# ethz-asl/aerial_mapper

Hardware: AMD Instinct MI355X
Metric: Mcells/s (DSM+ortho) (higher is better)
Workload: dtype f64

## Files before the change

### aerial_mapper_amd/csrc/amhip_api.hip

```cpp
#include <cmath>
#include <cstdio>
#include <cstdlib>
#include <cstring>
#include <limits>
#include <new>

#include "amhip_common.h"

namespace amhip {

static thread_local std::string g_last_error;

void set_last_error(const std::string& msg) { g_last_error = msg; }

int hip_fail(hipError_t e, const char* what, const char* file, int line) {
  char buf[512];
  std::snprintf(buf, sizeof(buf), "HIP error %d (%s) in `%s` at %s:%d", (int)e,
                hipGetErrorString(e), what, file, line);
  set_last_error(buf);
  return e == hipErrorOutOfMemory ? AMHIP_ERR_NOMEM : AMHIP_ERR_HIP;
}

static int arg_fail(const char* msg) {
  set_last_error(msg);
// ... 576 lines not shown
    ay = c.cone_ay;
    if (!tuning_on("no_distorted_prune")) p.r_in = c.cone_rin;
    if (tuning_on("distorted_square_cull")) ax = ay = cone;
  }
  if (have_cone) {
    p.cull = 1;
    double l[3] = {1.0, 0.0, ax}, r[3] = {-1.0, 0.0, ax};
    double t[3] = {0.0, 1.0, ay}, b[3] = {0.0, -1.0, ay};
    normalize3(l);
    normalize3(r);
    normalize3(t);
    normalize3(b);
    for (int k = 0; k < 3; ++k) {
      p.pl[0][k] = l[k];
      p.pl[1][k] = r[k];
      p.pl[2][k] = t[k];
      p.pl[3][k] = b[k];
    }
  } else if (p.cull) {
    const double W = cam.width, H = cam.height;
    double l[3] = {cam.fu, 0.0, cam.cu};
    double r[3] = {-cam.fu, 0.0, W - cam.cu};
    double t[3] = {0.0, cam.fv, cam.cv};
    double b[3] = {0.0, -cam.fv, H - cam.cv};
    normalize3(l);
    normalize3(r);
    normalize3(t);
    normalize3(b);
    for (int k = 0; k < 3; ++k) {
      p.pl[0][k] = l[k];
      p.pl[1][k] = r[k];
      p.pl[2][k] = t[k];
      p.pl[3][k] = b[k];
    }
  }
  *out = p;
}

static float layer_init_value(int layer) {
  switch (layer) {
    case AMHIP_LAYER_ORTHO:
      return 255.0f;
    case AMHIP_LAYER_ELEVATION_ANGLE:
    case AMHIP_LAYER_NUM_OBSERVATIONS:
      return 0.0f;
    default:
      return std::numeric_limits<float>::quiet_NaN();
  }
}

static int use_device(Ctx* c) {
  AMHIP_TRY(hipSetDevice(c->device));
  return AMHIP_OK;
}

static int fetch_status(Ctx* c) {
  AMHIP_TRY(hipMemcpyAsync(c->host_err, c->dev_err, sizeof(unsigned),
                           hipMemcpyDeviceToHost, c->stream));
  AMHIP_TRY(hipMemsetAsync(c->dev_err, 0, sizeof(unsigned), c->stream));
  AMHIP_TRY(hipStreamSynchronize(c->stream));
  const unsigned e = *c->host_err;
  if (e & kDevErrExactHit) {
    set_last_error(
        "a point coincides with a cell centre (reference: dsm.cc:165 "
        "CHECK(distances[i] > 0.0))");
    return AMHIP_ERR_EXACT_HIT;
  }
  if (e & kDevErrAlphaNonPos) {
    set_last_error(
        "observation angle alpha <= 0 (reference: ortho-backward-grid.cc:178 "
        "CHECK(alpha > 0.0))");
    return AMHIP_ERR_ALPHA_NONPOS;
  }
  if (e & kDevErrRectifyZeroW) {
    set_last_error("rectification: w == 0 (reference: rectifier.cpp:93,99 CHECK_NE(xyw(2), 0.0))");
    return AMHIP_ERR_ARG;
  }
  if (e & kDevErrHaloOverflow) {
    set_last_error(
        "tiled DSM: more halo points for a neighbouring window than send rows were reserved "
        "(cap_per_dest): the elevation near that edge is incomplete");
    return AMHIP_ERR_HALO_OVERFLOW;
  }
  return AMHIP_OK;
}

__global__ void k_halo_overflow_check(const unsigned long long* __restrict__ counts, int nd,
                                      unsigned long long cap, unsigned* __restrict__ dev_err) {
  if ((int)threadIdx.x < nd && counts[threadIdx.x] > cap) atomicOr(dev_err, kDevErrHaloOverflow);
}

static bool valid_layer(int l) { return l >= 0 && l < AMHIP_NUM_LAYERS; }

}

using namespace amhip;

extern "C" {

int amhip_abi_version(void) { return AMHIP_ABI_VERSION; }

const char* amhip_last_error(void) { return g_last_error.c_str(); }

void amhip_make_grid(double length_x, double length_y, double resolution,
                     double pos_x, double pos_y, amhip_grid_desc* out) {
  if (!out) return;
  out->rows = static_cast<int>(std::round(length_x / resolution));
  out->cols = static_cast<int>(std::round(length_y / resolution));
  out->resolution = resolution;
  out->length_x = static_cast<double>(out->rows) * resolution;
  out->length_y = static_cast<double>(out->cols) * resolution;
  out->pos_x = pos_x;
  out->pos_y = pos_y;
}

void amhip_cell_position(const amhip_grid_desc* grid, int i, int j, double* x,
                         double* y) {
  double bx, by;
  grid_bases(*grid, &bx, &by);
  if (x) *x = bx + grid->resolution * (-static_cast<double>(i));
  if (y) *y = by + grid->resolution * (-static_cast<double>(j));
}

int amhip_ctx_create(const amhip_grid_desc* grid, int device, amhip_ctx** out) {
  if (!grid) return arg_fail("amhip_ctx_create: null argument");
  return amhip_ctx_create_window(grid, 0, 0, grid->rows, grid->cols, device, out);
}

int amhip_ctx_create_window(const amhip_grid_desc* grid, int i0, int j0, int rows, int cols,
                            int device, amhip_ctx** out) {
  if (!grid || !out) return arg_fail("amhip_ctx_create: null argument");
  if (grid->rows <= 0 || grid->cols <= 0 || !(grid->resolution > 0.0))
    return arg_fail("amhip_ctx_create: empty grid");
  if (i0 < 0 || j0 < 0 || rows <= 0 || cols <= 0 || i0 + rows > grid->rows ||
      j0 + cols > grid->cols)
    return arg_fail("amhip_ctx_create_window: window outside the map");
  *out = nullptr;
  int ndev = 0;
  if (hipGetDeviceCount(&ndev) != hipSuccess || ndev <= 0) {
    (void)hipGetLastError();
    set_last_error("no HIP device visible (libaerial_mapper_hip needs a gfx950 GPU)");
    return AMHIP_ERR_NO_DEVICE;
  }
  if (device < 0 || device >= ndev) return arg_fail("amhip_ctx_create: bad device index");
  amhip_ctx* h = new (std::nothrow) amhip_ctx();
  if (!h) return AMHIP_ERR_NOMEM;
  Ctx* c = &h->impl;
  c->grid = *grid;
  c->device = device;
  c->win_i0 = i0;
  c->win_j0 = j0;
  c->win_rows = rows;
  c->win_cols = cols;
  c->cells = static_cast<size_t>(rows) * static_cast<size_t>(cols);
  {
    c->dsm_exact = amhip_default_dsm_precision() == AMHIP_DSM_EXACT ? 1 : 0;
  }
  int rc = AMHIP_OK;
  do {
    if ((rc = use_device(c))) break;
    if (hipStreamCreateWithFlags(&c->own_stream, hipStreamNonBlocking) != hipSuccess) {
      rc = hip_fail(hipGetLastError(), "hipStreamCreate", __FILE__, __LINE__);
      break;
    }
    c->stream = c->own_stream;
    hipError_t e = hipSuccess;
    for (int l = 0; l < AMHIP_NUM_LAYERS && e == hipSuccess; ++l)
      e = hipMalloc(reinterpret_cast<void**>(&c->layers[l]), c->cells * sizeof(float));
    if (e == hipSuccess) e = hipMalloc(reinterpret_cast<void**>(&c->dev_err), 4 * sizeof(unsigned));
    if (e == hipSuccess)
      e = hipMalloc(reinterpret_cast<void**>(&c->dev_zrange), 4 * sizeof(unsigned long long));
    if (e == hipSuccess)
      e = hipHostMalloc(reinterpret_cast<void**>(&c->host_err), sizeof(unsigned), 0);
    if (e == hipSuccess) {
      e = hipHostMalloc(reinterpret_cast<void**>(&c->host_tile_stats), 8 * sizeof(unsigned), 0);
      if (e == hipSuccess) std::memset(c->host_tile_stats, 0, 8 * sizeof(unsigned));
    }
    if (e == hipSuccess) {
      e = hipHostMalloc(reinterpret_cast<void**>(&c->host_sort_stats), 4 * sizeof(unsigned), 0);
      if (e == hipSuccess) std::memset(c->host_sort_stats, 0xFF, 4 * sizeof(unsigned));
    }
    if (e == hipSuccess) e = hipMalloc(reinterpret_cast<void**>(&c->dev_tickets), 16 * sizeof(unsigned));
    if (e == hipSuccess) e = hipMemsetAsync(c->dev_tickets, 0, 16 * sizeof(unsigned), c->stream);
    if (e == hipSuccess) e = hipMalloc(reinterpret_cast<void**>(&c->dev_bbox), 8 * sizeof(int));
    if (e == hipSuccess) e = hipHostMalloc(reinterpret_cast<void**>(&c->host_bbox), 8 * sizeof(int), 0);
    if (e == hipSuccess) e = hipMemsetAsync(c->dev_err, 0, sizeof(unsigned), c->stream);
    if (e != hipSuccess) {
      rc = hip_fail(e, "context allocation", __FILE__, __LINE__);
      break;
    }
    rc = amhip_layers_reset(h);
  } while (0);
  if (rc != AMHIP_OK) {
    const std::string keep = g_last_error;
    amhip_ctx_destroy(h);
    set_last_error(keep);
    return rc;
  }
  *out = h;
  return AMHIP_OK;
}

void amhip_ctx_destroy(amhip_ctx* h) {
  if (!h) return;
  Ctx* c = &h->impl;
  (void)hipSetDevice(c->device);
  if (c->stream) (void)hipStreamSynchronize(c->stream);
  drain_timers(c);
  for (TimedRegion& r : c->free_regions) {
    (void)hipEventDestroy(r.a);
    (void)hipEventDestroy(r.b);
  }
  for (int l = 0; l < AMHIP_NUM_LAYERS; ++l)
    if (c->layers[l]) (void)hipFree(c->layers[l]);
  void* bufs[] = {c->dev_bbox, c->ortho_list, c->zpart, c->dev_zrange, c->tile_list, c->tile_occ, c->fill_mask, c->stage_values, c->dev_err, c->sorted,       c->rank,        c->bin_start, c->bin_z, c->rec_a, c->rec_b, c->rec16, c->sidx, c->zref, c->zall, c->tmp_points, c->stripe_ws,
                  c->scan_partials, c->stage_points, c->frame_poses, c->stage_frames, c->stereo_ws};
  for (void* b : bufs)
    if (b) (void)hipFree(b);
  jpeg_scratch_free(&c->jpeg);
  if (c->host_err) (void)hipHostFree(c->host_err);
  if (c->host_tile_stats) (void)hipHostFree(c->host_tile_stats);
  if (c->host_sort_stats) (void)hipHostFree(c->host_sort_stats);
  if (c->dev_tickets) (void)hipFree(c->dev_tickets);
  if (c->host_bbox) (void)hipHostFree(c->host_bbox);
  if (c->order_event) (void)hipEventDestroy(c->order_event);
  if (c->own_stream) (void)hipStreamDestroy(c->own_stream);
  delete h;
}

int amhip_ctx_set_dsm_precision(amhip_ctx* h, int mode) {
  if (!h) return arg_fail("null context");
  if (mode != AMHIP_DSM_FAST && mode != AMHIP_DSM_EXACT) return arg_fail("unknown DSM precision mode");
  h->impl.dsm_exact = mode == AMHIP_DSM_EXACT ? 1 : 0;
  return AMHIP_OK;
}

int amhip_ctx_set_dsm_knn(amhip_ctx* h, int k) {
  if (!h) return arg_fail("null context");
  if (k < 0 || k > 8) return arg_fail("amhip_ctx_set_dsm_knn: k must be 0 (off) .. 8");
  h->impl.dsm_knn = k;
  return AMHIP_OK;
}

int amhip_ctx_set_stream(amhip_ctx* h, void* hip_stream) {
  if (!h) return arg_fail("null context");
  Ctx* c = &h->impl;
  int rc = use_device(c);
  if (rc) return rc;
  AMHIP_TRY(hipStreamSynchronize(c->stream));
  c->stream = hip_stream ? static_cast<hipStream_t>(hip_stream) : c->own_stream;
  return AMHIP_OK;
}

int amhip_ctx_synchronize(amhip_ctx* h) {
  if (!h) return arg_fail("null context");
  Ctx* c = &h->impl;
  int rc = use_device(c);
  if (rc) return rc;
  return fetch_status(c);
}

int amhip_layers_reset(amhip_ctx* h) {
  if (!h) return arg_fail("null context");
  Ctx* c = &h->impl;
  int rc = use_device(c);
  if (rc) return rc;
  const bool eager = tuning_on("eager_reset");
  {
    static const unsigned long long empty[2] = {0xFFF0000000000000ull, 0x000FFFFFFFFFFFFFull};
    AMHIP_TRY(hipMemcpyAsync(c->dev_zrange, empty, sizeof(empty), hipMemcpyHostToDevice, c->stream));
    c->zrange_valid = true;
  }
  for (int l = 0; l < AMHIP_NUM_LAYERS; ++l) {
    unsigned char& st = c->layer_state[l];
    if (st == 0 || st == 3) continue;
    if (st == 1 && !eager) {
      st = 3;
      continue;
    }
    if ((rc = launch_fill(c, c->layers[l], c->cells, layer_init_value(l)))) return rc;
    if (st == 1) st = 0;
  }
  return AMHIP_OK;
}

static int materialize(Ctx* c, int layer) {
  if (c->layer_state[layer] != 3) return AMHIP_OK;
  const int rc = launch_fill(c, c->layers[layer], c->cells, layer_init_value(layer));
  if (rc) return rc;
  c->layer_state[layer] = 0;
  return AMHIP_OK;
}

static void dirty_full(Ctx* c) {
  c->dirty_on_device = false;
  c->dirty[0] = c->dirty[1] = 0;
  c->dirty[2] = c->win_rows;
  c->dirty[3] = c->win_cols;
}

static int touch(Ctx* c, int layer) {
  dirty_full(c);
  const int rc = materialize(c, layer);
  if (rc) return rc;
  if (c->layer_state[layer] == 0) c->layer_state[layer] = 1;
  return AMHIP_OK;
// ... 526 lines not shown
                                        observation_index, colored_ortho};
  for (int l = 0; l < AMHIP_NUM_LAYERS; ++l)
    if (ups[l]) {
      overwrite(c, l);
      AMHIP_TRY(hipMemcpyAsync(c->layers[l], ups[l], bytes, hipMemcpyHostToDevice,
                               c->stream));
    }
  const size_t row = (size_t)cam->width * (size_t)channels;
  const size_t frame = row * (size_t)cam->height;
  if ((rc = ensure_capacity(&c->stage_frames, &c->stage_frames_cap, frame * F))) return rc;
  for (size_t f = 0; f < F; ++f) {
    if (!images[f]) return arg_fail("null image");
    if (steps[f] < row) return arg_fail("image step smaller than a row");
    if (steps[f] == row)
      AMHIP_TRY(hipMemcpyAsync(c->stage_frames + f * frame, images[f], frame,
                               hipMemcpyHostToDevice, c->stream));
    else
      AMHIP_TRY(hipMemcpy2DAsync(c->stage_frames + f * frame, row, images[f], steps[f],
                                 row, (size_t)cam->height, hipMemcpyHostToDevice,
                                 c->stream));
  }
  if ((rc = amhip_ortho_backward_process_dev(h, cam, host_T_G_C, F, c->stage_frames,
                                             frame, row, channels, colored)))
    return rc;
  float* downs[AMHIP_NUM_LAYERS] = {ortho,           nullptr,
                                    elevation_angle, num_observations,
                                    observation_index, colored_ortho};
  for (int l = 0; l < AMHIP_NUM_LAYERS; ++l)
    if (downs[l]) {
      if ((rc = materialize(c, l))) return rc;
      AMHIP_TRY(hipMemcpyAsync(downs[l], c->layers[l], bytes, hipMemcpyDeviceToHost,
                               c->stream));
    }
  return fetch_status(c);
}


int amhip_ctx_enable_timing(amhip_ctx* h, int on) {
  if (!h) return arg_fail("null context");
  h->impl.timing = on != 0;
  return AMHIP_OK;
}

int amhip_ctx_timing_reset(amhip_ctx* h) {
  if (!h) return arg_fail("null context");
  Ctx* c = &h->impl;
  int rc = use_device(c);
  if (rc) return rc;
  drain_timers(c);
  for (int k = 0; k < AMHIP_NUM_KERNELS; ++k) {
    c->slot_ms[k] = 0.0;
    c->slot_launches[k] = 0;
  }
  return AMHIP_OK;
}

int amhip_ctx_kernel_time(amhip_ctx* h, int kernel, double* total_ms,
                          int64_t* launches) {
  if (!h || kernel < 0 || kernel >= AMHIP_NUM_KERNELS) return arg_fail("bad kernel slot");
  Ctx* c = &h->impl;
  int rc = use_device(c);
  if (rc) return rc;
  drain_timers(c);
  if (total_ms) *total_ms = c->slot_ms[kernel];
  if (launches) *launches = c->slot_launches[kernel];
  return AMHIP_OK;
}

const char* amhip_kernel_name(int kernel) {
  switch (kernel) {
    case AMHIP_K_DSM_BIN_COUNT:
      return "k_dsm_p3_count";
    case AMHIP_K_DSM_SCATTER:
      return "k_dsm_p3_scatter";
    case AMHIP_K_DSM_SCAN:
      return "k_dsm_p3_place";
    case AMHIP_K_DSM_GATHER:
      return "k_dsm_gather";
    case AMHIP_K_ORTHO:
      return "k_ortho_backward";
    case AMHIP_K_MISC:
      return "memset/fill";
    case AMHIP_K_HALO_SELECT:
      return "k_halo_select";
    case AMHIP_K_STEREO:
      return "k_stereo";
    default:
      return "?";
  }
}

int amhip_set_tuning(const char* key, double value) {
  if (!tuning_set(key, value)) return arg_fail("amhip_set_tuning: unknown key (include/aerial_mapper_hip.h lists them)");
  return AMHIP_OK;
}

double amhip_get_tuning(const char* key, double dflt) { return key ? tuning(key, dflt) : dflt; }

int amhip_default_dsm_precision(void) {
  const char* fast = std::getenv("AMHIP_DSM_FAST");
  return (fast && fast[0] && fast[0] != '0' && !std::getenv("AMHIP_DSM_EXACT")) ? AMHIP_DSM_FAST : AMHIP_DSM_EXACT;
}

int amhip_ctx_order_after(amhip_ctx* h, void* other_stream) {
  if (!h) return arg_fail("null context");
  Ctx* c = &h->impl;
  int rc = use_device(c);
  if (rc) return rc;
  hipStream_t other = static_cast<hipStream_t>(other_stream);
  if (other == c->stream) return AMHIP_OK;
  if (!c->order_event) AMHIP_TRY(hipEventCreateWithFlags(&c->order_event, hipEventDisableTiming));
  AMHIP_TRY(hipEventRecord(c->order_event, c->stream));
  AMHIP_TRY(hipStreamWaitEvent(other, c->order_event, 0));
  return AMHIP_OK;
}

int amhip_ctx_dsm_gather_stats(amhip_ctx* h, int64_t* out8) {
  if (!h || !out8) return arg_fail("amhip_ctx_dsm_gather_stats: null argument");
  Ctx* c = &h->impl;
  int rc = use_device(c);
  if (rc) return rc;
  for (int k = 0; k < 8; ++k) out8[k] = 0;
  if (!c->tile_list || c->last_ntiles == 0) return AMHIP_OK;
  unsigned hdr[8];
  AMHIP_TRY(hipMemcpyAsync(hdr, c->tile_list, sizeof(hdr), hipMemcpyDeviceToHost, c->stream));
  AMHIP_TRY(hipStreamSynchronize(c->stream));
  for (int k = 0; k < 7; ++k) out8[k] = hdr[k];
  out8[4] += hdr[7];
  out8[7] = c->last_ntiles;
  return AMHIP_OK;
}

int amhip_ctx_dsm_stats(amhip_ctx* h, int64_t* points_binned, int64_t* num_bins,
                        int32_t* bin_cells) {
  if (!h) return arg_fail("null context");
  Ctx* c = &h->impl;
  int rc = use_device(c);
  if (rc) return rc;
  if (points_binned) {
    *points_binned = 0;
    if (c->bin_start && c->last_num_bins > 0) {
      uint32_t total = 0;
      AMHIP_TRY(hipMemcpyAsync(&total, c->bin_start + c->last_num_bins,
                               sizeof(uint32_t), hipMemcpyDeviceToHost, c->stream));
      AMHIP_TRY(hipStreamSynchronize(c->stream));
      *points_binned = total;
    }
  }
  if (num_bins) *num_bins = c->last_num_bins;
  if (bin_cells) *bin_cells = c->last_bin_cells;
  return AMHIP_OK;
}

}
```

### aerial_mapper_amd/csrc/amhip_common.h

```cpp
#ifndef AMHIP_COMMON_H_
#define AMHIP_COMMON_H_

#include <hip/hip_runtime.h>

#include <cstddef>
#include <cstdint>
#include <string>
#include <vector>

#include "aerial_mapper_hip.h"
#include "amhip_tuning.h"
#include "amhip_ortho_fold.h"

namespace amhip {

void set_last_error(const std::string& msg);
int hip_fail(hipError_t e, const char* what, const char* file, int line);

#define AMHIP_TRY(expr)                                                  \
  do {                                                                   \
    hipError_t _e = (expr);                                              \
    if (_e != hipSuccess) return ::amhip::hip_fail(_e, #expr, __FILE__, __LINE__); \
  } while (0)

constexpr int kMaxLevels = 24;
constexpr int kMaxW0 = 16;

struct DsmParams {
  double base_x, base_y, res;
  int rows, cols;
  int i_off, j_off;
  double sub_x, sub_y;
  int pcl_mode;
  int only_unfilled;
  double inv_res;
  int B, M, nbx, nby;
  int nlevels;
  double T[kMaxLevels];
  int w[kMaxLevels];
  int lds_ok;
  int p3_r1;
  int p3_c, p3_w;
  int p3_n1, p3_n2;
  int p3_cap;
  unsigned mul_B, mul_r1, mul_w;
  int wr[2 * kMaxW0 + 1];
  int wr2[2 * kMaxW0 + 2];
  int wrp[kMaxW0 + 1];
  int lds_cap;
  int lds_cells;
  int tile_j;
  int tiles_i, tiles_j;
  unsigned lds_bytes;
  int knn_k;
  int fx_ok;
  int fx_S;
  float fx_thi, fx_tlo;
  float fx_denmax;
  float fx_epsw;
  unsigned lds_bytes_f32;
  int canon_all;
  int out_i0, out_j0, out_pitch;
};

struct PtsView {
  const double* sorted;
  const uint4* rec;
  const uint32_t* sidx;
  const double* cloud;
  const double* zref;
  double sub_x, sub_y;
};


struct OrthoParams {
  double base_x, base_y, res;
  int rows, cols;
  int i_off, j_off;
  double fu, fv, cu, cv;
  double dist[4];
  int width, height, distortion;
  int num_frames;
  int channels, colored;
  size_t frame_stride, row_step;
  double pl[4][3];
  int cull;
  int virt_out, virt_nobs;
  int coarse;
  int fast;
  FoldCam fold;
  int prune;
  double radius_scale;
  double r_in;
};

enum : unsigned { kDevErrExactHit = 1u, kDevErrAlphaNonPos = 2u, kDevErrHaloOverflow = 4u,
                  kDevErrRectifyZeroW = 8u };

constexpr int kMaxHaloDests = 8;
struct HaloParams {
  double base_x, base_y, inv_res, sub_x, sub_y;
  int nd;
  double lo_i[kMaxHaloDests], hi_i[kMaxHaloDests], lo_j[kMaxHaloDests], hi_j[kMaxHaloDests];
  unsigned long long cap;
  unsigned long long off[kMaxHaloDests], cap_d[kMaxHaloDests];
  double in_lo_i, in_hi_i, in_lo_j, in_hi_j;
};
struct SortSplit {
  int phase;
  size_t n_prefix;
  HaloParams hp;
  double* halo_out;
  unsigned long long* halo_counts;
};

struct JpegScratch {
  uint8_t* dev = nullptr;
  size_t cap = 0;
  uint8_t* pinned = nullptr;
  uint8_t* image = nullptr;
  size_t image_cap = 0;
  uint8_t* out = nullptr;
  size_t out_cap = 0;
};
enum { kJpegGray8 = 0, kJpegBgr8 = 1, kJpegBgr16s = 2 };
struct JpegSource {
  const void* dev;
  size_t step;
  int width, height;
  int mode;
};
void jpeg_scratch_free(JpegScratch* ws);
int jpeg_scratch_image(JpegScratch* ws, size_t bytes, uint8_t** out);
int jpeg_encode_run(hipStream_t stream, JpegScratch* ws, const JpegSource& src, int quality,
                    uint8_t* dev_out, size_t cap, size_t* bytes);
int jpeg_write_run(const char* what, hipStream_t stream, JpegScratch* ws, const JpegSource& src,
                   int quality, const char* filename);

struct TimedRegion {
  hipEvent_t a, b;
  int slot;
};

struct Ctx {
  amhip_grid_desc grid;
  int win_i0 = 0, win_j0 = 0;
  int win_rows = 0, win_cols = 0;
  int device = 0;
  hipStream_t own_stream = nullptr;
  hipStream_t stream = nullptr;
  hipEvent_t order_event = nullptr;
  size_t cells = 0;
  int dsm_exact = 0;
  int dsm_exact_now = 0;
  int rough_hold = 0;
  bool last_call_f32 = false;
  int dsm_knn = 0;

  float* layers[AMHIP_NUM_LAYERS] = {nullptr, nullptr, nullptr,
                                     nullptr, nullptr, nullptr};
  unsigned char layer_state[AMHIP_NUM_LAYERS] = {1, 1, 1, 1, 1, 1};
  unsigned long long* dev_zrange = nullptr;
  bool zrange_valid = false;
  double* zpart = nullptr;
  size_t zpart_cap = 0;
  unsigned* dev_err = nullptr;
  unsigned* host_err = nullptr;

  PtsView pts = {};
  double* sorted = nullptr;
  size_t sorted_cap = 0;
  uint32_t* rank = nullptr;
  size_t rank_cap = 0;
  uint32_t* bin_start = nullptr;
  size_t bin_cap = 0;
  uint32_t* rec_a = nullptr;
  size_t rec_a_cap = 0;
  uint32_t* rec_b = nullptr;
  size_t rec_b_cap = 0;
  uint32_t* rec16 = nullptr;
  size_t rec16_cap = 0;
  uint32_t* sidx = nullptr;
  size_t sidx_cap = 0;
  double* zref = nullptr;
  size_t zref_cap = 0;
  double* zall = nullptr;
  size_t zall_cap = 0;
  uint32_t* bin_z = nullptr;
  size_t bin_z_cap = 0;
  bool bin_z_valid = false;
  uint32_t* scan_partials = nullptr;
  size_t partial_cap = 0;
  double* tmp_points = nullptr;
  size_t tmp_points_cap = 0;
  uint32_t* stripe_ws = nullptr;
  size_t stripe_ws_cap = 0;
  uint8_t* tile_occ = nullptr;
  size_t tile_occ_cap = 0;
  int* tile_list = nullptr;
  size_t tile_list_cap = 0;
  unsigned char* fill_mask = nullptr;
  size_t fill_mask_cap = 0;
  int32_t* stage_values = nullptr;
  size_t stage_values_cap = 0;
  double* stage_points = nullptr;
  size_t stage_points_cap = 0;

  amhip_camera cone_cam = {};
  double cone = 0.0;
  int cone_state = 0;
  int cone_state_rect = 0;
  double cone_rect_cone = 0.0, cone_ax = 0.0, cone_ay = 0.0, cone_rin = 0.0;
  FramePose* frame_poses = nullptr;
  size_t frame_pose_cap = 0;
  uint8_t* stage_frames = nullptr;
  size_t stage_frames_cap = 0;
  int dirty[4] = {0, 0, 0, 0};
  bool dirty_on_device = false;
  int* dev_bbox = nullptr;
  int* host_bbox = nullptr;
  int* ortho_list = nullptr;
  size_t ortho_list_cap = 0;

  bool tiled_pending = false;
  const double* tiled_xyz = nullptr;
  size_t tiled_n = 0;
  int tiled_radius_sq = 0;
  double tiled_ce = 0.0, tiled_cn = 0.0;
  SortSplit tiled_split = {};
  DsmParams tiled_params = {};

  int64_t last_points_binned = 0;
  int64_t last_num_bins = 0;
  int32_t last_bin_cells = 0;
  int64_t last_ntiles = 0;
  uint32_t* aux_zero_words = nullptr;
  int aux_nzero = 0;
  bool aux_done = false;
  size_t range_parts = 0;
  unsigned long long* range_running = nullptr;
  unsigned* dev_tickets = nullptr;
  unsigned* host_sort_stats = nullptr;
  unsigned long long sort_stats_sig = 0, tile_stats_sig = 0;
  unsigned* host_tile_stats = nullptr;

  uint8_t* stereo_ws = nullptr;
  size_t stereo_ws_cap = 0;
  JpegScratch jpeg;

  bool timing = false;
  std::vector<TimedRegion> regions;
  std::vector<TimedRegion> free_regions;
  double slot_ms[AMHIP_NUM_KERNELS] = {};
  int64_t slot_launches[AMHIP_NUM_KERNELS] = {};
};

struct ScopedTimer {
  Ctx* c;
  TimedRegion r;
  bool on;
  ScopedTimer(Ctx* ctx, int slot);
  ~ScopedTimer();
};

template <typename T>
int ensure_capacity(T** ptr, size_t* cap, size_t need);

int ensure_bytes(void** ptr, size_t* cap_bytes, size_t need_bytes);

int launch_fill(Ctx* c, float* dst, size_t n, float value);

struct DensifyParams {
  int width, height;
  size_t disp_step, img_step;
  double Q03, Q11, Q13, Q23, Q32;
  double R[9], t[3];
};
inline DensifyParams densify_params(const double* K, double baseline, const double* R_G_C,
                                    const double* t_G_C1, int width, int height, size_t disp_step,
                                    size_t img_step) {
  DensifyParams p = {};
  p.width = width;
  p.height = height;
  p.disp_step = disp_step;
  p.img_step = img_step;
  const double fx = K[0], fy = K[4], cx = K[2], cy = K[5];
  p.Q03 = -cx;
  p.Q11 = fx / fy;
  p.Q13 = -cy * (fx / fy);
  p.Q23 = fx;
  p.Q32 = 1.0 / baseline;
  for (int k = 0; k < 9; ++k) p.R[k] = R_G_C[k];
  for (int k = 0; k < 3; ++k) p.t[k] = t_G_C1[k];
  return p;
}
int densify_run(Ctx* c, const DensifyParams& p, const float* dev_disparity,
                const uint8_t* dev_image_left, double* dev_xyz_out, int32_t* dev_intensity_out,
                size_t capacity, long long* dev_count);

struct SeqState {
  unsigned long long running, base;
  unsigned pairs, skip;
};
int densify_append_run(Ctx* c, const DensifyParams& p, const float* dev_disparity,
                       const uint8_t* dev_image_left, double* dev_xyz, int32_t* dev_intensities,
                       size_t capacity, SeqState* dev_state, void* dev_pc2, bool replace,
                       const unsigned* dev_err_word = nullptr);
struct BatchStrides {
  size_t left, right, mask, disp, raw;
};
struct StereoImages {
  const uint8_t* left;
  size_t left_step;
  const uint8_t* right;
  size_t right_step;
  const uint8_t* mask;
  size_t mask_step;
  float* disp;
  size_t disp_step;
  int16_t* raw;
  size_t raw_step;
  int batch;
  BatchStrides bs;
};
int stereo_params_check(const amhip_stereo_settings& s, int width, int height);
int stereo_scratch_reserve(Ctx* c, const amhip_stereo_settings& s, int width, int height, int batch);
int stereo_match(Ctx* c, const amhip_stereo_settings& s, int width, int height, const StereoImages& im);
int undistort_frames_run(hipStream_t stream, const amhip_camera& cam, const uint8_t* dev_frames,
                         size_t frame_stride, size_t row_step, int channels, int G, uint8_t* dev_out);

int halo_select_run(Ctx* c, const double* dev_xyz, size_t n, const HaloParams& hp,
                    double* dev_out, unsigned long long* dev_counts);
constexpr int kBboxBias = 1 << 30;
int dsm_bbox_run(Ctx* c, const double* dev_xyz, size_t n, const DsmParams& p, int* dev_bbox5);
int make_halo_params(const Ctx& c, double center_easting, double center_northing,
                     const int32_t* dest_windows, int nd, double margin_m, size_t cap_per_dest,
                     HaloParams* out);
bool no_launch_skips();
int dsm_sort(Ctx* c, const double* dev_xyz, const int32_t* dev_values, size_t n,
             const DsmParams& p, unsigned long long* zrange, const SortSplit* split = nullptr);
int dsm_run(Ctx* c, const double* dev_xyz, const int32_t* dev_values, size_t n,
            const DsmParams& p, float* out, unsigned char* mask, unsigned* unfilled,
            bool fill_untouched = false, float init_value = 0.0f,
            unsigned long long* zrange = nullptr, const SortSplit* split = nullptr);
int ortho_run(Ctx* c, const OrthoParams& p, const FramePose* dev_poses, const FrameFast* dev_fast,
              const uint8_t* dev_frames);

int ctx_last_dirty(Ctx* c, int rect[4]);
int ctx_use_device(Ctx* c);
int ctx_materialize(Ctx* c, int layer);
void ctx_overwrite(Ctx* c, int layer);
int ctx_layer_set_initial(Ctx* c, int layer);
int ctx_fetch_status(Ctx* c);
float ctx_layer_init_value(int layer);
bool ctx_layer_is_initial(const Ctx* c, int layer);
int arg_failure(const char* msg);

struct HPose {
  double qw, qx, qy, qz, tx, ty, tz;
};
HPose hpose_from7(const double* p);
HPose hpose_inverse(const HPose& T);
HPose hpose_compose(const HPose& A, const HPose& B);

}

struct amhip_ctx {
  amhip::Ctx impl;
};

#endif
```

### aerial_mapper_amd/csrc/amhip_sort.hip

```cpp
#include <algorithm>
#include <cstdlib>

#include "amhip_common.h"
#include "amhip_device.h"

namespace amhip {

constexpr uint32_t kNoRank = 0xFFFFFFFFu;

__device__ __forceinline__ int div_by(int n, int d, unsigned m) {
  if (m == 0u) return n;
  if (m == 0xFFFFFFFFu) return n / d;
  return (int)__umulhi((unsigned)n, m);
}

__device__ __forceinline__ bool point_bin(const DsmParams& p, double px,
                                          double py, uint32_t* bin) {
  const double cx = (p.base_x - px) * p.inv_res - (double)p.i_off;
  const double cy = (p.base_y - py) * p.inv_res - (double)p.j_off;
  const double lo = -(double)p.M - 0.5;
  const double hx = (double)(p.rows + p.M) - 0.5;
  const double hy = (double)(p.cols + p.M) - 0.5;
  if (!(cx >= lo && cx < hx && cy >= lo && cy < hy)) return false;
  int ix = (int)floor(cx + 0.5) + p.M;
// ... 236 lines not shown
          if (zall) {
            zlo = fmin(zlo, z[u]);
            zhi = fmax(zhi, z[u]);
          }
        }
        if (kHalo && halo_candidate(hp, x[u], y[u])) look |= 1u << u;
      }
    }
    if (kHalo) {
#pragma nounroll
      while (look) {
        const int u = __builtin_ctz(look);
        look &= look - 1;
        halo_emit(stage, hp, xyz, base + (size_t)u * stride, halo_out, halo_counts);
      }
    }
  }
  if (kHalo) halo_flush(stage, hp, xyz, halo_out, halo_counts);
  if (zall)
    range_commit_wave(zlo, zhi, zall, (size_t)blockIdx.x * (kP3CountThreads / 64) + (threadIdx.x >> 6));
  __syncthreads();
  uint32_t* row = hist_rows + (size_t)blockIdx.x * nk;
  for (int k = threadIdx.x; k < nk; k += kP3CountThreads) row[k] = s_hist[k];
}

struct SortAux {
  unsigned long long* call_range;
  uint32_t* zero_words;
  int nzero;
};
__device__ __forceinline__ void aux_reset(const SortAux& a) {
  if (threadIdx.x == 0 && a.call_range) {
    a.call_range[0] = kOrderedPlusInf;
    a.call_range[1] = kOrderedMinusInf;
  }
  if (a.zero_words && (int)threadIdx.x < a.nzero) a.zero_words[threadIdx.x] = 0u;
}

__device__ __forceinline__ void
p3_scan_body(const uint32_t* __restrict__ cnt, int n1, int n2,
              uint32_t* __restrict__ start2, uint32_t* __restrict__ cursor2,
              uint32_t* __restrict__ start1, uint32_t* __restrict__ cursor1,
              uint32_t* __restrict__ blk2, unsigned cap_small, unsigned cap_big,
              uint32_t* __restrict__ big_list, unsigned chunk,
              unsigned* __restrict__ host_big ) {
  __shared__ unsigned lds[1024 / 64 + 1];
  __shared__ unsigned s_start1[kP3MaxKeys + 1];
  const int nk = n1 * n2;
  unsigned carry = 0;
  if (threadIdx.x == 0) big_list[0] = 0;
  __syncthreads();
  constexpr int kMaxIt = 32;
  {
    const int lane = threadIdx.x & 63, wid = threadIdx.x >> 6;
    const int seg = ((nk + 16 * 64 - 1) / (16 * 64)) * 64;
    const int iters = seg / 64;
    const int w0 = wid * seg;
    unsigned v[kMaxIt];
#pragma unroll
    for (int q = 0; q < kMaxIt; ++q) {
      const int i = w0 + q * 64 + lane;
      v[q] = (q < iters && i < nk) ? cnt[i] : 0u;
    }
    unsigned run = 0;
#pragma unroll
    for (int q = 0; q < kMaxIt; ++q) {
      if (q < iters) {
        if (v[q] > cap_small)
          big_list[1 + atomicAdd(&big_list[0], 1u)] = (uint32_t)(w0 + q * 64 + lane);
        const unsigned incl = wave_incl_scan(v[q], lane);
        v[q] = run + incl - v[q];
        run += __shfl(incl, 63, 64);
      }
    }
    if (lane == 0) lds[wid] = run;
    __syncthreads();
    unsigned base = 0, total = 0;
#pragma unroll
    for (int w = 0; w < 16; ++w) {
      const unsigned t = lds[w];
      if (w < wid) base += t;
      total += t;
    }
#pragma unroll
    for (int q = 0; q < kMaxIt; ++q) {
      const int i = w0 + q * 64 + lane;
      if (q < iters && i < nk) {
        const unsigned st = base + v[q];
        start2[i] = st;
        cursor2[i] = st;
        if (i % n2 == 0) s_start1[i / n2] = st;
      }
    }
    carry = total;
  }
  __syncthreads();
  if (threadIdx.x == 0) {
    start2[nk] = carry;
    s_start1[n1] = carry;
  }
  __syncthreads();
  const int k = threadIdx.x;
  unsigned nblk = 0;
  if (k < n1) {
    start1[k] = s_start1[k];
    cursor1[k] = s_start1[k];
    nblk = (s_start1[k + 1] - s_start1[k] + chunk - 1) / chunk;
  }
  if (k == 0) start1[n1] = carry;
  unsigned total;
  const unsigned ex = block_excl_scan<1024>(nblk, &total, lds);
  if (k < n1) blk2[k] = ex;
  if (k == 0) blk2[n1] = total;
  if (k == 0 && host_big) host_big[0] = big_list[0];
}

__global__ void __launch_bounds__(1024)
k_dsm_p3_reduce_scan(const uint32_t* __restrict__ hist_rows, int nrows, uint32_t* __restrict__ cnt, int n1, int n2,
                     uint32_t* __restrict__ start2, uint32_t* __restrict__ cursor2,
                     uint32_t* __restrict__ start1, uint32_t* __restrict__ cursor1,
                     uint32_t* __restrict__ blk2, unsigned cap_small, unsigned cap_big,
                     uint32_t* __restrict__ big_list, unsigned chunk,
                     SortAux aux, unsigned* __restrict__ host_big, unsigned* __restrict__ ticket) {
  __shared__ uint32_t s_part[16][64];
  __shared__ unsigned s_last;
  const int nk = n1 * n2;
  const int lane = threadIdx.x & 63, wid = threadIdx.x >> 6;
  const int k = blockIdx.x * 64 + lane;
  uint32_t sum = 0;
  if (k < nk)
    for (int r = wid; r < nrows; r += 16) sum += hist_rows[(size_t)r * nk + k];
  s_part[wid][lane] = sum;
  __syncthreads();
  if (wid == 0 && k < nk) {
    uint32_t t = 0;
#pragma unroll
    for (int w = 0; w < 16; ++w) t += s_part[w][lane];
    cnt[k] = t;
  }
  __syncthreads();
  if (threadIdx.x == 0) {
    __threadfence();
    s_last = atomicAdd(ticket, 1u) == gridDim.x - 1u ? 1u : 0u;
  }
  __syncthreads();
  if (!s_last) return;
  __threadfence();
  if (threadIdx.x == 0) *ticket = 0u;
  aux_reset(aux);
  p3_scan_body(cnt, n1, n2, start2, cursor2, start1, cursor1, blk2, cap_small, cap_big, big_list, chunk, host_big);
}


template <bool kFirst>
__device__ __forceinline__ void p3_scatter_body(const unsigned vb, const double* __restrict__ src,
                                                const int32_t* __restrict__ values, size_t n,
                                                const DsmParams& p, const uint32_t* __restrict__ start1,
                                                const uint32_t* __restrict__ blk2,
                                                uint32_t* __restrict__ cursor, double* __restrict__ dst,
                                                double* __restrict__ zpart) {
  extern __shared__ double s_pts[];
  uint32_t* s_dest = reinterpret_cast<uint32_t*>(s_pts + 3 * kP3Chunk);
  uint32_t* s_cnt = s_dest + kP3Chunk;
  uint32_t* s_off = s_cnt + kP3MaxKeys;
  uint32_t* s_base = s_off + kP3MaxKeys;
  uint32_t* s_scan = s_base + kP3MaxKeys;
  const int tid = threadIdx.x;
  int nkeys;
  size_t c0, c1;
  if (kFirst) {
    c0 = (size_t)vb * kP3Chunk;
    c1 = min(c0 + (size_t)kP3Chunk, n);
    nkeys = p.p3_n1;
  } else {
    const int n1 = p.p3_n1;
    const uint32_t b = vb;
    if (b >= blk2[n1]) return;
    int lo = 0, hi = n1;
    while (hi - lo > 1) {
      const int mid = (lo + hi) >> 1;
      if (blk2[mid] <= b) lo = mid; else hi = mid;
    }
    c0 = (size_t)start1[lo] + (size_t)(b - blk2[lo]) * kP3Chunk;
    c1 = min(c0 + (size_t)kP3Chunk, (size_t)start1[lo + 1]);
    nkeys = p.p3_n2;
    cursor += (size_t)lo * p.p3_n2;
  }
  if (tid < kP3MaxKeys) s_cnt[tid] = 0;
  __syncthreads();
  double px[kP3PerThread], py[kP3PerThread], pz[kP3PerThread];
  double zlo = __builtin_huge_val(), zhi = -__builtin_huge_val();
  uint32_t slot[kP3PerThread];
  if (c1 <= c0) return;
#pragma unroll
  for (int k = 0; k < kP3PerThread; ++k) {
    const size_t ld = min(c0 + tid + (size_t)k * kP3Threads, c1 - 1);
    px[k] = src[3 * ld + 0];
    py[k] = src[3 * ld + 1];
    pz[k] = src[3 * ld + 2];
  }
  if (kFirst && values) {
#pragma unroll
    for (int k = 0; k < kP3PerThread; ++k)
      pz[k] = (double)values[min(c0 + tid + (size_t)k * kP3Threads, c1 - 1)];
  }
#pragma unroll
  for (int k = 0; k < kP3PerThread; ++k) {
    const size_t idx = c0 + tid + (size_t)k * kP3Threads;
    slot[k] = 0xFFFFFFFFu;
    if (idx < c1) {
      double x = px[k], y = py[k];
      const double z = pz[k];
      if (kFirst) {
        x -= p.sub_x;
        y -= p.sub_y;
      }
      px[k] = x;
      py[k] = y;
      int k1, k2;
      if (p3_keys(p, x, y, &k1, &k2)) {
        const int key = kFirst ? k1 : k2;
        slot[k] = ((uint32_t)key << 13) | atomicAdd(&s_cnt[key], 1u);
        if (kFirst) {
          zlo = fmin(zlo, z);
          zhi = fmax(zhi, z);
        }
      }
    }
  }
  if (kFirst && zpart)
    range_commit_wave(zlo, zhi, zpart, (size_t)vb * (kP3Threads / 64) + (tid >> 6));
  __syncthreads();
  unsigned my_base = 0;
  {
    const unsigned c = (tid < nkeys) ? s_cnt[tid] : 0u;
    unsigned total;
    const unsigned ex = block_excl_scan<kP3Threads>(c, &total, s_scan);
    if (tid < nkeys) {
      s_off[tid] = ex;
      if (c) my_base = atomicAdd(&cursor[tid], c);
    }
    if (tid == 0) s_scan[23] = total;
  }
  __syncthreads();
#pragma unroll
  for (int k = 0; k < kP3PerThread; ++k) {
    if (slot[k] != 0xFFFFFFFFu) {
      const uint32_t key = slot[k] >> 13, rank = slot[k] & 0x1FFFu;
      const uint32_t q = s_off[key] + rank;
      s_pts[3 * q + 0] = px[k];
      s_pts[3 * q + 1] = py[k];
      s_pts[3 * q + 2] = pz[k];
      s_dest[q] = slot[k];
    }
  }
  if (tid < nkeys) s_base[tid] = my_base;
  __syncthreads();
  const uint32_t ne = 3u * s_scan[23];
  for (uint32_t e = tid; e < ne; e += kP3Threads) {
    const uint32_t q = e / 3u;
    const uint32_t d = s_dest[q];
    const uint32_t b = s_base[d >> 13];
    dst[3 * (size_t)(b + (d & 0x1FFFu)) + (e - 3u * q)] = s_pts[e];
  }
}

template <bool kFirst>
__global__ void __launch_bounds__(kP3Threads)
k_dsm_p3_scatter(const double* __restrict__ src, const int32_t* __restrict__ values, size_t n,
                 DsmParams p, const uint32_t* __restrict__ start1,
                 const uint32_t* __restrict__ blk2, uint32_t* __restrict__ cursor,
                 double* __restrict__ dst, double* __restrict__ zpart) {
  p3_scatter_body<kFirst>(blockIdx.x, src, values, n, p, start1, blk2, cursor, dst, zpart);
}

__device__ __forceinline__ uint32_t place_zkey(double z) {
  const uint32_t b = __float_as_uint((float)z);
  return (b >> 31) ? ~b : (b | 0x80000000u);
}
template <int THREADS, int PER>
__device__ __forceinline__ void place_subpartition(const double* __restrict__ src, const DsmParams& p,
                                                   int cap, const uint32_t* __restrict__ start2,
                                                   uint32_t* __restrict__ bin_start,
                                                   double* __restrict__ sorted, int sp,
                                                   unsigned skip_lo, unsigned skip_hi,
                                                   uint2* __restrict__ bin_z) {
  extern __shared__ double s_pts[];
  uint32_t* s_bins = reinterpret_cast<uint32_t*>(s_pts + 3 * cap);
  uint32_t* s_scan = s_bins + p.p3_w;
  uint32_t* s_zlo = s_scan + 24;
  uint32_t* s_zhi = s_zlo + p.p3_w;
  const int tid = threadIdx.x;
  const int k1 = sp / p.p3_n2, k2 = sp - k1 * p.p3_n2;
  const int rr = k2 / p.p3_c;
  const int row = k1 * p.p3_r1 + rr;
  const int bx0 = (k2 - rr * p.p3_c) * p.p3_w;
  const int nbw = min(p.p3_w, p.nbx - bx0);
  if (sp == 0 && tid == 0)
    bin_start[(size_t)p.nbx * p.nby] = start2[p.p3_n1 * p.p3_n2];
  if (row >= p.nby || nbw <= 0) return;
  const uint32_t g0 = start2[sp], g1 = start2[sp + 1];
  for (int k = tid; k < nbw; k += THREADS) {
    s_bins[k] = 0;
    if (bin_z) {
      s_zlo[k] = 0xFFFFFFFFu;
      s_zhi[k] = 0u;
    }
  }
  __syncthreads();
  if ((g1 - g0) > skip_lo && (g1 - g0) <= skip_hi) return;
  const bool in_lds = (int)(g1 - g0) <= cap && cap <= THREADS * PER;
  double px[PER], py[PER], pz[PER];
  int pb[PER];
  if (in_lds) {
    if (g1 > g0) {
#pragma unroll
      for (int k = 0; k < PER; ++k) {
        const size_t ld = min(g0 + tid + (uint32_t)k * THREADS, g1 - 1);
        px[k] = src[3 * ld + 0];
        py[k] = src[3 * ld + 1];
        pz[k] = src[3 * ld + 2];
      }
    }
#pragma unroll
    for (int k = 0; k < PER; ++k) {
      const uint32_t idx = g0 + tid + (uint32_t)k * THREADS;
      pb[k] = -1;
      if (idx < g1) {
        int bx, by;
        point_bin_xy(p, px[k], py[k], &bx, &by);
        pb[k] = bx - bx0;
        atomicAdd(&s_bins[pb[k]], 1u);
        if (bin_z) {
          const uint32_t zk = place_zkey(pz[k]);
          atomicMin(&s_zlo[pb[k]], zk);
          atomicMax(&s_zhi[pb[k]], zk);
        }
      }
    }
  } else {
    for (uint32_t idx = g0 + tid; idx < g1; idx += THREADS) {
      int bx, by;
      point_bin_xy(p, src[3 * (size_t)idx + 0], src[3 * (size_t)idx + 1], &bx, &by);
      atomicAdd(&s_bins[bx - bx0], 1u);
    }
  }
  __syncthreads();
  {
    const int per = (nbw + THREADS - 1) / THREADS;
    const int lo = tid * per;
    const int hi = min(lo + per, nbw);
    unsigned sum = 0;
    for (int k = lo; k < hi; ++k) sum += s_bins[k];
    unsigned total;
    unsigned run = block_excl_scan<THREADS>(sum, &total, s_scan);
    for (int k = lo; k < hi; ++k) {
      const unsigned t = s_bins[k];
      s_bins[k] = run;
      run += t;
    }
  }
  __syncthreads();
  uint32_t* out_start = bin_start + (size_t)row * p.nbx + bx0;
  for (int k = tid; k < nbw; k += THREADS) out_start[k] = g0 + s_bins[k];
  if (bin_z && in_lds) {
    uint2* zrow = bin_z + (size_t)row * p.nbx + bx0;
    for (int k = tid; k < nbw; k += THREADS) zrow[k] = make_uint2(s_zlo[k], s_zhi[k]);
  }
  __syncthreads();
  if (!in_lds) {
    for (uint32_t idx = g0 + tid; idx < g1; idx += THREADS) {
      const double x = src[3 * (size_t)idx + 0];
      const double y = src[3 * (size_t)idx + 1];
      const double z = src[3 * (size_t)idx + 2];
      int bx, by;
      point_bin_xy(p, x, y, &bx, &by);
      const size_t o = (size_t)g0 + atomicAdd(&s_bins[bx - bx0], 1u);
      sorted[3 * o + 0] = x;
      sorted[3 * o + 1] = y;
      sorted[3 * o + 2] = z;
      if (bin_z) {
        const uint32_t zk = place_zkey(z);
        atomicMin(&s_zlo[bx - bx0], zk);
        atomicMax(&s_zhi[bx - bx0], zk);
      }
    }
    if (bin_z) {
      __syncthreads();
      uint2* zrow = bin_z + (size_t)row * p.nbx + bx0;
      for (int k = tid; k < nbw; k += THREADS) zrow[k] = make_uint2(s_zlo[k], s_zhi[k]);
    }
    return;
  }
#pragma unroll
  for (int k = 0; k < PER; ++k) {
    if (pb[k] >= 0) {
      const uint32_t q = atomicAdd(&s_bins[pb[k]], 1u);
      s_pts[3 * q + 0] = px[k];
      s_pts[3 * q + 1] = py[k];
      s_pts[3 * q + 2] = pz[k];
    }
  }
  __syncthreads();
  const uint32_t ne = 3u * (g1 - g0);
  double* out = sorted + 3 * (size_t)g0;
  for (uint32_t e = tid; e < ne; e += THREADS) out[e] = s_pts[e];
}


template <int THREADS, bool kRec, int PER>
__device__ __forceinline__ void place_rounds(const void* __restrict__ src_v, const DsmParams& p, int cap,
                                             const uint32_t* __restrict__ start2,
                                             uint32_t* __restrict__ bin_start, double* __restrict__ sorted,
                                             uint4* __restrict__ rec16, uint32_t* __restrict__ sidx,
                                             uint2* __restrict__ bin_z, int sp) {
  extern __shared__ double s_pts_raw[];
  constexpr int kWordsPer = kRec ? 5 : 6;
  constexpr int kRegs = PER > 0 ? PER : 1;
  uint32_t* s_words = reinterpret_cast<uint32_t*>(s_pts_raw);
  uint32_t* s_bins = s_words + (size_t)kWordsPer * cap;
  uint32_t* s_cur = s_bins + p.p3_w + 1;
  uint32_t* s_scan = s_cur + p.p3_w;
  uint32_t* s_zlo = s_scan + 24;
  uint32_t* s_zhi = s_zlo + p.p3_w;
  const double* srcd = reinterpret_cast<const double*>(src_v);
  const uint32_t* srcw = reinterpret_cast<const uint32_t*>(src_v);
  const int tid = threadIdx.x;
  const int k1 = sp / p.p3_n2, k2 = sp - k1 * p.p3_n2;
  const int rr = k2 / p.p3_c;
  const int row = k1 * p.p3_r1 + rr;
  const int bx0 = (k2 - rr * p.p3_c) * p.p3_w;
  const int nbw = min(p.p3_w, p.nbx - bx0);
  if (row >= p.nby || nbw <= 0) return;
  const uint32_t g0 = start2[sp], g1 = start2[sp + 1];
  auto zkey = [](uint32_t fbits) { return (fbits >> 31) ? ~fbits : (fbits | 0x80000000u); };
  for (int k = tid; k <= nbw; k += THREADS) s_bins[k] = 0;
  if (bin_z)
    for (int k = tid; k < nbw; k += THREADS) {
      s_zlo[k] = 0xFFFFFFFFu;
      s_zhi[k] = 0u;
    }
  __syncthreads();
  auto bin_of = [&](uint32_t idx) -> int {
    if (kRec) return div_by((int)(srcw[(size_t)kRecWords * idx] & 0xFFFFu), p.B, p.mul_B) - bx0;
    int bx, by;
    point_bin_xy(p, srcd[3 * (size_t)idx + 0], srcd[3 * (size_t)idx + 1], &bx, &by);
    return bx - bx0;
  };
  double rx[kRegs], ry[kRegs], rz[kRegs];
  uint32_t rw[kRegs][kRecWords];
  int rb[kRegs];
  if (PER > 0) {
    if (g1 > g0) {
#pragma unroll
      for (int k = 0; k < kRegs; ++k) {
        const size_t ld = min(g0 + tid + (uint32_t)k * THREADS, g1 - 1);
        if (kRec) {
#pragma unroll
          for (int t = 0; t < kRecWords; ++t) rw[k][t] = srcw[(size_t)kRecWords * ld + t];
        } else {
          rx[k] = srcd[3 * ld + 0];
          ry[k] = srcd[3 * ld + 1];
          rz[k] = srcd[3 * ld + 2];
        }
      }
    }
#pragma unroll
    for (int k = 0; k < kRegs; ++k) {
      const uint32_t idx = g0 + tid + (uint32_t)k * THREADS;
      rb[k] = -1;
      if (idx < g1) {
        if (kRec) {
          rb[k] = div_by((int)(rw[k][0] & 0xFFFFu), p.B, p.mul_B) - bx0;
        } else {
          int bx, by;
          point_bin_xy(p, rx[k], ry[k], &bx, &by);
          rb[k] = bx - bx0;
        }
        atomicAdd(&s_bins[rb[k]], 1u);
        if (bin_z) {
          const uint32_t zk = kRec ? zkey(rw[k][3]) : place_zkey(rz[k]);
          atomicMin(&s_zlo[rb[k]], zk);
          atomicMax(&s_zhi[rb[k]], zk);
        }
      }
    }
  } else {
    for (uint32_t idx = g0 + tid; idx < g1; idx += THREADS) {
      const int b = bin_of(idx);
      atomicAdd(&s_bins[b], 1u);
      if (bin_z) {
        const uint32_t zk = kRec ? zkey(srcw[(size_t)kRecWords * idx + 3]) : place_zkey(srcd[3 * (size_t)idx + 2]);
        atomicMin(&s_zlo[b], zk);
        atomicMax(&s_zhi[b], zk);
      }
    }
  }
  __syncthreads();
  {
    const int per = (nbw + THREADS - 1) / THREADS;
    const int lo = tid * per;
    const int hi = min(lo + per, nbw);
    unsigned sum = 0;
    for (int k = lo; k < hi; ++k) sum += s_bins[k];
    unsigned total;
    unsigned run = block_excl_scan<THREADS>(sum, &total, s_scan);
    for (int k = lo; k < hi; ++k) {
      const unsigned t = s_bins[k];
      s_bins[k] = run;
      run += t;
    }
    if (tid == 0) s_bins[nbw] = total;
  }
  __syncthreads();
  {
    uint32_t* out_start = bin_start + (size_t)row * p.nbx + bx0;
    for (int k = tid; k < nbw; k += THREADS) out_start[k] = g0 + s_bins[k];
    if (bin_z) {
      uint2* zrow = bin_z + (size_t)row * p.nbx + bx0;
      for (int k = tid; k < nbw; k += THREADS) zrow[k] = make_uint2(s_zlo[k], s_zhi[k]);
    }
  }
  auto put = [&](bool direct, uint32_t q, uint32_t base, const uint32_t* v, double x, double y, double z) {
    if (kRec) {
      if (direct) {
        rec16[(size_t)g0 + q] = make_uint4(v[0], v[1], v[2], v[3]);
        sidx[(size_t)g0 + q] = v[4];
      } else {
#pragma unroll
        for (int t = 0; t < kRecWords; ++t) s_words[(size_t)kRecWords * (q - base) + t] = v[t];
      }
    } else {
      double* o = direct ? sorted + 3 * ((size_t)g0 + q) : s_pts_raw + 3 * (size_t)(q - base);
      o[0] = x;
      o[1] = y;
      o[2] = z;
    }
  };
  int lo_bin = 0;
  while (lo_bin < nbw) {
    const uint32_t base = s_bins[lo_bin];
    int a = lo_bin, b = nbw;
    while (b - a > 0) {
      const int mid = (a + b + 1) >> 1;
      if (s_bins[mid] - base <= (uint32_t)cap) a = mid; else b = mid - 1;
    }
    const bool direct = a == lo_bin;
    const int hi_bin = direct ? lo_bin + 1 : a;
    const uint32_t cnt = s_bins[hi_bin] - base;
    for (int k = lo_bin + tid; k < hi_bin; k += THREADS) s_cur[k] = s_bins[k];
    __syncthreads();
    if (PER > 0) {
#pragma unroll
      for (int k = 0; k < kRegs; ++k) {
        if (rb[k] >= lo_bin && rb[k] < hi_bin) {
          const uint32_t q = atomicAdd(&s_cur[rb[k]], 1u);
          put(direct, q, base, rw[k], rx[k], ry[k], rz[k]);
        }
      }
    } else {
      for (uint32_t idx = g0 + tid; idx < g1; idx += THREADS) {
        const int bb = bin_of(idx);
        if (bb < lo_bin || bb >= hi_bin) continue;
        const uint32_t q = atomicAdd(&s_cur[bb], 1u);
        uint32_t v[kRecWords] = {0u, 0u, 0u, 0u, 0u};
        double x = 0.0, y = 0.0, z = 0.0;
        if (kRec) {
#pragma unroll
          for (int t = 0; t < kRecWords; ++t) v[t] = srcw[(size_t)kRecWords * idx + t];
        } else {
          x = srcd[3 * (size_t)idx + 0];
          y = srcd[3 * (size_t)idx + 1];
          z = srcd[3 * (size_t)idx + 2];
        }
        put(direct, q, base, v, x, y, z);
      }
    }
    __syncthreads();
    if (!direct) {
      if (kRec) {
        for (uint32_t q = tid; q < cnt; q += THREADS) {
          const uint32_t* r = s_words + (size_t)kRecWords * q;
          rec16[(size_t)g0 + base + q] = make_uint4(r[0], r[1], r[2], r[3]);
          sidx[(size_t)g0 + base + q] = r[4];
        }
      } else {
        double* out = sorted + 3 * ((size_t)g0 + base);
        for (uint32_t e = tid; e < 3u * cnt; e += THREADS) out[e] = s_pts_raw[e];
      }
    }
    __syncthreads();
    lo_bin = hi_bin;
  }
}

__global__ void __launch_bounds__(kP3PlaceThreads)
k_dsm_p3_place(const double* __restrict__ src, DsmParams p, int cap,
               const uint32_t* __restrict__ start2, uint32_t* __restrict__ bin_start,
               double* __restrict__ sorted, unsigned skip_lo, unsigned skip_hi,
               uint2* __restrict__ bin_z,
               const uint32_t* __restrict__ big_list, unsigned* __restrict__ host_big) {
  if (host_big && blockIdx.x == 0 && threadIdx.x == 0) host_big[0] = big_list[0];
  place_subpartition<kP3PlaceThreads, kP3PlacePer>(src, p, cap, start2, bin_start, sorted,
                                                   (int)blockIdx.x, skip_lo, skip_hi, bin_z);
}

__global__ void __launch_bounds__(kP3BigThreads)
k_dsm_p3_place_big(const double* __restrict__ src, DsmParams p,
                   const uint32_t* __restrict__ start2, uint32_t* __restrict__ bin_start,
                   double* __restrict__ sorted, const uint32_t* __restrict__ big_list,
                   uint2* __restrict__ bin_z, int cap_rounds, unsigned rounds_above, unsigned reg_max) {
  const unsigned count = big_list[0];
  for (unsigned k = blockIdx.x; k < count; k += gridDim.x) {
    const int sp = (int)big_list[1 + k];
    const uint32_t cnt = start2[sp + 1] - start2[sp];
    if (cnt > rounds_above && cnt <= min(reg_max, (unsigned)(kP3BigThreads * kP3RoundsPer)))
      place_rounds<kP3BigThreads, false, kP3RoundsPer>(src, p, cap_rounds, start2, bin_start, sorted, nullptr,
                                                       nullptr, bin_z, sp);
    else if (cnt > rounds_above)
      place_rounds<kP3BigThreads, false, 0>(src, p, cap_rounds, start2, bin_start, sorted, nullptr, nullptr,
                                            bin_z, sp);
    else
      place_subpartition<kP3BigThreads, kP3BigPer>(src, p, kP3BigCap, start2, bin_start, sorted, sp, 0u,
                                                   0u, bin_z);
    __syncthreads();
  }
}

constexpr int kRecPerThread = 6;
constexpr int kRecChunk = kP3Threads * kRecPerThread;

__global__ void __launch_bounds__(1024)
k_dsm_zref(const double* __restrict__ part, size_t nparts, double* __restrict__ zref) {
  __shared__ double s_pair[2 * 16];
  double lo = __builtin_huge_val(), hi = -__builtin_huge_val();
  for (size_t k = threadIdx.x; k < nparts; k += 1024) {
    lo = fmin(lo, part[2 * k]);
    hi = fmax(hi, part[2 * k + 1]);
  }
#pragma unroll
  for (int d = 32; d > 0; d >>= 1) {
    lo = fmin(lo, __shfl_xor(lo, d, 64));
    hi = fmax(hi, __shfl_xor(hi, d, 64));
  }
  if ((threadIdx.x & 63) == 0) {
    s_pair[2 * (threadIdx.x >> 6)] = lo;
    s_pair[2 * (threadIdx.x >> 6) + 1] = hi;
  }
  __syncthreads();
  if (threadIdx.x == 0) {
    for (int w = 1; w < 16; ++w) {
      lo = fmin(lo, s_pair[2 * w]);
      hi = fmax(hi, s_pair[2 * w + 1]);
    }
    const bool ok = lo <= hi && lo > -1.0e300 && hi < 1.0e300;
    zref[0] = ok ? 0.5 * lo + 0.5 * hi : 0.0;
    zref[1] = lo;
    zref[2] = hi;
  }
}

__device__ __forceinline__ bool make_record(const DsmParams& p, double px, double py, double z,
                                            double zref, uint32_t row, uint32_t* w) {
  const double cx = (p.base_x - px) * p.inv_res - (double)p.i_off;
  const double cy = (p.base_y - py) * p.inv_res - (double)p.j_off;
  const double lo = -(double)p.M - 0.5;
  const double hx = (double)(p.rows + p.M) - 0.5;
  const double hy = (double)(p.cols + p.M) - 0.5;
  if (!(cx >= lo && cx < hx && cy >= lo && cy < hy)) return false;
  int ix = (int)floor(cx + 0.5) + p.M;
  int iy = (int)floor(cy + 0.5) + p.M;
  ix = min(max(ix, 0), p.rows + 2 * p.M - 1);
  iy = min(max(iy, 0), p.cols + 2 * p.M - 1);
  const double scale = (double)(1u << p.fx_S);
  const double fx = (cx + (double)p.M) - (double)ix;
  const double fy = (cy + (double)p.M) - (double)iy;
  w[0] = (uint32_t)ix | ((uint32_t)iy << 16);
  w[1] = (uint32_t)(int)rint(fx * scale);
  w[2] = (uint32_t)(int)rint(fy * scale);
  w[3] = __float_as_uint((float)(z - zref));
  w[4] = row;
  return true;
}

__device__ __forceinline__ void record_keys(const DsmParams& p, uint32_t w0, int* k1, int* k2,
                                            int* bx_out) {
  const int bx = div_by((int)(w0 & 0xFFFFu), p.B, p.mul_B);
  const int by = div_by((int)(w0 >> 16), p.B, p.mul_B);
  const int a = div_by(by, p.p3_r1, p.mul_r1);
  *k1 = a;
  *k2 = (by - a * p.p3_r1) * p.p3_c + div_by(bx, p.p3_w, p.mul_w);
  *bx_out = bx;
}

template <bool kFirst>
__global__ void __launch_bounds__(kP3Threads)
k_dsm_p3_scatter_rec(const double* __restrict__ cloud, const uint32_t* __restrict__ src, size_t n,
                     DsmParams p, const double* __restrict__ zref,
                     const uint32_t* __restrict__ start1, const uint32_t* __restrict__ blk2,
                     uint32_t* __restrict__ cursor, uint32_t* __restrict__ dst,
                     double* __restrict__ zpart) {
  extern __shared__ uint32_t s_words[];
  uint32_t* s_dest = s_words + kRecWords * kRecChunk;
  uint32_t* s_cnt = s_dest + kRecChunk;
  uint32_t* s_off = s_cnt + kP3MaxKeys;
  uint32_t* s_base = s_off + kP3MaxKeys;
  uint32_t* s_scan = s_base + kP3MaxKeys;
  const int tid = threadIdx.x;
  int nkeys;
  size_t c0, c1;
  if (kFirst) {
    c0 = (size_t)blockIdx.x * kRecChunk;
    c1 = min(c0 + (size_t)kRecChunk, n);
    nkeys = p.p3_n1;
  } else {
    const int n1 = p.p3_n1;
    const uint32_t b = blockIdx.x;
    if (b >= blk2[n1]) return;
    int lo = 0, hi = n1;
    while (hi - lo > 1) {
      const int mid = (lo + hi) >> 1;
      if (blk2[mid] <= b) lo = mid; else hi = mid;
    }
    c0 = (size_t)start1[lo] + (size_t)(b - blk2[lo]) * kRecChunk;
    c1 = min(c0 + (size_t)kRecChunk, (size_t)start1[lo + 1]);
    nkeys = p.p3_n2;
    cursor += (size_t)lo * p.p3_n2;
  }
  if (tid < kP3MaxKeys) s_cnt[tid] = 0;
  __syncthreads();
  const double zr = kFirst ? zref[0] : 0.0;
  uint32_t w[kRecPerThread][kRecWords];
  double zlo = __builtin_huge_val(), zhi = -__builtin_huge_val();
  uint32_t slot[kRecPerThread];
  if (c1 <= c0) return;
  double cx[kFirst ? kRecPerThread : 1], cy[kFirst ? kRecPerThread : 1], cz[kFirst ? kRecPerThread : 1];
#pragma unroll
  for (int k = 0; k < kRecPerThread; ++k) {
    const size_t ld = min(c0 + tid + (size_t)k * kP3Threads, c1 - 1);
    if (kFirst) {
      cx[k] = cloud[3 * ld + 0];
      cy[k] = cloud[3 * ld + 1];
      cz[k] = cloud[3 * ld + 2];
    } else {
#pragma unroll
      for (int q = 0; q < kRecWords; ++q) w[k][q] = src[kRecWords * ld + q];
    }
  }
#pragma unroll
  for (int k = 0; k < kRecPerThread; ++k) {
    const size_t idx = c0 + tid + (size_t)k * kP3Threads;
    slot[k] = 0xFFFFFFFFu;
    if (idx < c1) {
      bool in;
      if (kFirst) {
        const double x = cx[k] - p.sub_x;
        const double y = cy[k] - p.sub_y;
        const double z = cz[k];
        in = make_record(p, x, y, z, zr, (uint32_t)idx, w[k]);
        if (in) {
          zlo = fmin(zlo, z);
          zhi = fmax(zhi, z);
        }
      } else {
        in = true;
      }
      if (in) {
        int k1, k2, bx;
        record_keys(p, w[k][0], &k1, &k2, &bx);
        const int key = kFirst ? k1 : k2;
        slot[k] = ((uint32_t)key << 13) | atomicAdd(&s_cnt[key], 1u);
      }
    }
  }
  if (kFirst && zpart)
    range_commit_wave(zlo, zhi, zpart, (size_t)blockIdx.x * (kP3Threads / 64) + (tid >> 6));
  __syncthreads();
// ... 254 lines not shown
    w[2] = lo_j;
    w[3] = hi_j;
    w[4] = (int)cnt;
  }
  __syncthreads();
  if (threadIdx.x == 0) {
    unsigned total = 0;
    for (int k = 0; k < 4; ++k) {
      lo_i = min(lo_i, s_box[k][0]);
      hi_i = max(hi_i, s_box[k][1]);
      lo_j = min(lo_j, s_box[k][2]);
      hi_j = max(hi_j, s_box[k][3]);
      total += (unsigned)s_box[k][4];
    }
    if (total) {
      atomicMax(&out5[0], kBboxBias - lo_i);
      atomicMax(&out5[1], hi_i + kBboxBias);
      atomicMax(&out5[2], kBboxBias - lo_j);
      atomicMax(&out5[3], hi_j + kBboxBias);
      atomicAdd(reinterpret_cast<unsigned*>(&out5[4]), total);
    }
  }
}

int dsm_bbox_run(Ctx* c, const double* dev_xyz, size_t n, const DsmParams& p, int* dev_bbox5) {
  ScopedTimer t(c, AMHIP_K_DSM_BIN_COUNT);
  AMHIP_TRY(hipMemsetAsync(dev_bbox5, 0, 5 * sizeof(int), c->stream));
  size_t grid = std::min<size_t>((n + 2047) / 2048, 128);
  hipLaunchKernelGGL(k_dsm_bbox, dim3((unsigned)grid), dim3(256), 0, c->stream, dev_xyz, n, p, dev_bbox5);
  AMHIP_TRY(hipGetLastError());
  return AMHIP_OK;
}

constexpr int kScanT = 256;
constexpr int kScanI = 16;
constexpr int kScanE = kScanT * kScanI;

__global__ void __launch_bounds__(kScanT)
k_scan_partials(const uint32_t* __restrict__ in, size_t n,
                uint32_t* __restrict__ partials) {
  __shared__ unsigned lds[kScanT / 64 + 1];
  const size_t base = (size_t)blockIdx.x * kScanE + (size_t)threadIdx.x * kScanI;
  unsigned s = 0;
  if (base + kScanI <= n) {
    const uint4* v = reinterpret_cast<const uint4*>(in + base);
#pragma unroll
    for (int k = 0; k < kScanI / 4; ++k) {
      const uint4 q = v[k];
      s += q.x + q.y + q.z + q.w;
    }
  } else {
    for (int k = 0; k < kScanI; ++k)
      if (base + k < n) s += in[base + k];
  }
  unsigned total;
  (void)block_excl_scan<kScanT>(s, &total, lds);
  if (threadIdx.x == 0) partials[blockIdx.x] = total;
}

__global__ void __launch_bounds__(1024)
k_scan_top(uint32_t* __restrict__ partials, size_t nb,
           uint32_t* __restrict__ total_out, SortAux aux) {
  __shared__ unsigned lds[1024 / 64 + 1];
  aux_reset(aux);
  unsigned carry = 0;
  for (size_t base = 0; base < nb; base += 1024) {
    const size_t i = base + threadIdx.x;
    const unsigned v = (i < nb) ? partials[i] : 0u;
    unsigned total;
    const unsigned ex = block_excl_scan<1024>(v, &total, lds);
    if (i < nb) partials[i] = carry + ex;
    carry += total;
  }
  if (threadIdx.x == 0) *total_out = carry;
}

__global__ void __launch_bounds__(kScanT)
k_scan_final(uint32_t* __restrict__ data, size_t n,
             const uint32_t* __restrict__ partials) {
  __shared__ unsigned lds[kScanT / 64 + 1];
  const size_t base = (size_t)blockIdx.x * kScanE + (size_t)threadIdx.x * kScanI;
  unsigned v[kScanI];
  const bool full = base + kScanI <= n;
  if (full) {
    const uint4* src = reinterpret_cast<const uint4*>(data + base);
#pragma unroll
    for (int k = 0; k < kScanI / 4; ++k) {
      const uint4 q = src[k];
      v[4 * k + 0] = q.x;
      v[4 * k + 1] = q.y;
      v[4 * k + 2] = q.z;
      v[4 * k + 3] = q.w;
    }
  } else {
#pragma unroll
    for (int k = 0; k < kScanI; ++k) v[k] = (base + k < n) ? data[base + k] : 0u;
  }
  unsigned s = 0;
#pragma unroll
  for (int k = 0; k < kScanI; ++k) s += v[k];
  unsigned total;
  unsigned run = block_excl_scan<kScanT>(s, &total, lds) + partials[blockIdx.x];
#pragma unroll
  for (int k = 0; k < kScanI; ++k) {
    const unsigned t = v[k];
    v[k] = run;
    run += t;
  }
  if (full) {
    uint4* dst = reinterpret_cast<uint4*>(data + base);
#pragma unroll
    for (int k = 0; k < kScanI / 4; ++k)
      dst[k] = make_uint4(v[4 * k], v[4 * k + 1], v[4 * k + 2], v[4 * k + 3]);
  } else {
#pragma unroll
    for (int k = 0; k < kScanI; ++k)
      if (base + k < n) data[base + k] = v[k];
  }
}


static void p3_rounds_knob(int* cap_rounds, unsigned* rounds_above, unsigned* reg_max) {
  const int knob = (int)tuning("p3_rounds_cap", 0.0);
  const bool reread = tuning_on("p3_rounds_reread");
  if (knob >= 16 && knob < *cap_rounds) {
    *cap_rounds = knob;
    *rounds_above = (unsigned)knob;
  }
  if (reread) *reg_max = 0u;
}

bool no_launch_skips() {
  return tuning_on("no_launch_skips");
}

static unsigned long long sort_geometry_signature(const DsmParams& p) {
  unsigned long long h = 1469598103934665603ull;
  auto mix = [&](const void* v, size_t bytes) {
    const unsigned char* b = static_cast<const unsigned char*>(v);
    for (size_t k = 0; k < bytes; ++k) h = (h ^ b[k]) * 1099511628211ull;
  };
  const int ints[] = {p.rows, p.cols, p.M, p.B, p.nbx, p.nby, p.i_off, p.j_off, p.p3_r1, p.p3_c,
                      p.p3_w, p.p3_n1, p.p3_n2, p.p3_cap};
  const double dbls[] = {p.base_x, p.base_y, p.res, p.inv_res, p.sub_x, p.sub_y};
  mix(ints, sizeof(ints));
  mix(dbls, sizeof(dbls));
  return h ? h : 1ull;
}


static int dsm_sort_impl(Ctx* c, const double* dev_xyz, const int32_t* dev_values, size_t n,
                         const DsmParams& p, unsigned long long* zrange, const SortSplit* split);

int dsm_sort(Ctx* c, const double* dev_xyz, const int32_t* dev_values, size_t n,
             const DsmParams& p, unsigned long long* zrange, const SortSplit* split) {
  const int rc = dsm_sort_impl(c, dev_xyz, dev_values, n, p, zrange, split);
  if (rc) return rc;
  if (!c->aux_done && !(split && split->phase == 1)) return arg_failure("dsm_sort: the call's range was not reset");
  return AMHIP_OK;
}

static int dsm_sort_impl(Ctx* c, const double* dev_xyz, const int32_t* dev_values, size_t n,
                         const DsmParams& p, unsigned long long* zrange, const SortSplit* split) {
  double* zpart = nullptr;
  {
    const size_t max_waves = 8 * std::max<size_t>((n + 2047) / 2048 + 1, 256 * 16);
    const int rc = ensure_capacity(&c->zpart, &c->zpart_cap, 2 * max_waves + 16);
    if (rc) return rc;
    zpart = c->zpart;
  }
  const SortAux aux = {c->dev_zrange + 2, c->aux_zero_words, c->aux_zero_words ? c->aux_nzero : 0};
  c->aux_done = false;
  c->range_parts = 0;
  c->range_running = zrange;
  const size_t nbins = (size_t)p.nbx * (size_t)p.nby;
  const size_t nblocks_scan = (nbins + kScanE - 1) / kScanE;
  const bool force_one_level_ = tuning_on("sort_one_level");
  const unsigned long long geo_sig = sort_geometry_signature(p);
  {
    int rc;
    if ((rc = ensure_capacity(&c->sorted, &c->sorted_cap, 3 * n))) return rc;
    if ((rc = ensure_capacity(&c->bin_start, &c->bin_cap, nbins + 4))) return rc;
  }
  c->last_num_bins = (int64_t)nbins;
  c->last_bin_cells = p.B;
  c->bin_z_valid = false;
  c->pts = PtsView{c->sorted, nullptr, nullptr, dev_xyz, nullptr, p.sub_x, p.sub_y};
  const bool rec = p.fx_ok && !p.pcl_mode && !dev_values;
  if (rec) {
    int rc;
    if ((rc = ensure_capacity(&c->rec16, &c->rec16_cap, 4 * n + 16))) return rc;
    if ((rc = ensure_capacity(&c->sidx, &c->sidx_cap, n + 16))) return rc;
    if ((rc = ensure_capacity(&c->zref, &c->zref_cap, (size_t)8))) return rc;
  }

  const bool force_one_level = force_one_level_;
  const bool three_pass = p.p3_n1 > 0 && !force_one_level;
  if (split && split->phase == 1 && !three_pass)
    return halo_select_run(c, dev_xyz, split->n_prefix, split->hp, split->halo_out,
                           split->halo_counts);
  if (split && !three_pass) split = nullptr;
  if (three_pass) {
    const int n1 = p.p3_n1, n2 = p.p3_n2, nk = n1 * n2;
    auto count_grid = [](size_t len) {
      return std::min<size_t>(std::max<size_t>((len + 8191) / 8192, 1), 256);
    };
    const size_t n_a = split ? split->n_prefix : n;
    const size_t g_a = count_grid(n_a), g_b = n > n_a ? count_grid(n - n_a) : 0;
    const size_t gcount = g_a + g_b;
    int rc;
    if (rec) {
      if ((rc = ensure_capacity(&c->rec_a, &c->rec_a_cap, (size_t)kRecWords * n + 16))) return rc;
      if ((rc = ensure_capacity(&c->rec_b, &c->rec_b_cap, (size_t)kRecWords * n + 16))) return rc;
      if ((rc = ensure_capacity(&c->zall, &c->zall_cap, 2 * gcount * (kP3CountThreads / 64) + 16))) return rc;
    } else if ((rc = ensure_capacity(&c->tmp_points, &c->tmp_points_cap, 3 * n))) {
      return rc;
    }
    double* const zall = rec ? c->zall : nullptr;
    const size_t ws_words = gcount * (size_t)nk + 4 * (size_t)nk + 4 * (size_t)n1 + 64;
    if ((rc = ensure_capacity(&c->stripe_ws, &c->stripe_ws_cap, ws_words))) return rc;
    uint32_t* hist_rows = c->stripe_ws;
    uint32_t* cnt = hist_rows + gcount * (size_t)nk;
    uint32_t* start2 = cnt + nk;
    uint32_t* cursor2 = start2 + nk + 1;
    uint32_t* start1 = cursor2 + nk;
    uint32_t* cursor1 = start1 + n1 + 1;
    uint32_t* blk2 = cursor1 + n1;
    uint32_t* big_list = blk2 + n1 + 1;
    {
      ScopedTimer t(c, AMHIP_K_DSM_BIN_COUNT);
      const size_t lds = (size_t)nk * sizeof(uint32_t);
      const size_t lds_halo = (size_t)((nk + 1) & ~1) * sizeof(uint32_t) + sizeof(HaloStage);
      AMHIP_TRY(hipFuncSetAttribute(reinterpret_cast<const void*>(k_dsm_p3_count<false>),
                                    hipFuncAttributeMaxDynamicSharedMemorySize, (int)lds));
      AMHIP_TRY(hipFuncSetAttribute(reinterpret_cast<const void*>(k_dsm_p3_count<true>),
                                    hipFuncAttributeMaxDynamicSharedMemorySize, (int)lds_halo));
      const HaloParams no_halo = {};
      if (split && split->phase == 1) {
        AMHIP_TRY(hipMemsetAsync(split->halo_counts, 0,
                                 sizeof(unsigned long long) * split->hp.nd, c->stream));
        hipLaunchKernelGGL(k_dsm_p3_count<true>, dim3((unsigned)g_a), dim3(kP3CountThreads),
                           lds_halo, c->stream, dev_xyz, n_a, p, hist_rows, split->hp, split->halo_out,
                           split->halo_counts, zall);
        AMHIP_TRY(hipGetLastError());
        return AMHIP_OK;
      }
      if (!split)
        hipLaunchKernelGGL(k_dsm_p3_count<false>, dim3((unsigned)g_a), dim3(kP3CountThreads), lds,
                           c->stream, dev_xyz, n_a, p, hist_rows, no_halo, (double*)nullptr,
                           (unsigned long long*)nullptr, zall);
      else if (g_b)
        hipLaunchKernelGGL(k_dsm_p3_count<false>, dim3((unsigned)g_b), dim3(kP3CountThreads), lds,
                           c->stream, dev_xyz + 3 * n_a, n - n_a, p, hist_rows + g_a * (size_t)nk,
                           no_halo, (double*)nullptr, (unsigned long long*)nullptr,
                           zall ? zall + 2 * g_a * (kP3CountThreads / 64) : nullptr);
      if (rec)
        hipLaunchKernelGGL(k_dsm_zref, dim3(1), dim3(1024), 0, c->stream, zall,
                           (split && !g_b ? g_a : gcount) * (size_t)(kP3CountThreads / 64), c->zref);
      hipLaunchKernelGGL(k_dsm_p3_reduce_scan, dim3((unsigned)((nk + 63) / 64)), dim3(1024), 0, c->stream,
                         hist_rows, (int)gcount, cnt, n1, n2, start2, cursor2, start1, cursor1, blk2,
                         (unsigned)p.p3_cap, (unsigned)kP3BigCap, big_list, (unsigned)(rec ? kRecChunk : kP3Chunk),
                         aux, (unsigned*)nullptr, c->dev_tickets);
      c->aux_done = true;
      AMHIP_TRY(hipGetLastError());
    }
    if (rec) {
      {
        ScopedTimer t(c, AMHIP_K_DSM_SCATTER);
        const size_t lds = (size_t)kRecChunk * (kRecWords + 1) * 4 + (3 * kP3MaxKeys + 32) * sizeof(uint32_t);
        AMHIP_TRY(hipFuncSetAttribute(reinterpret_cast<const void*>(k_dsm_p3_scatter_rec<true>),
                                      hipFuncAttributeMaxDynamicSharedMemorySize, (int)lds));
        AMHIP_TRY(hipFuncSetAttribute(reinterpret_cast<const void*>(k_dsm_p3_scatter_rec<false>),
                                      hipFuncAttributeMaxDynamicSharedMemorySize, (int)lds));
        const size_t g1 = (n + kRecChunk - 1) / kRecChunk;
        hipLaunchKernelGGL(k_dsm_p3_scatter_rec<true>, dim3((unsigned)g1), dim3(kP3Threads), lds,
                           c->stream, dev_xyz, (const uint32_t*)nullptr, n, p, c->zref, start1, blk2,
                           cursor1, c->rec_a, zpart);
        c->range_parts = (size_t)g1 * (kP3Threads / 64);
        hipLaunchKernelGGL(k_dsm_p3_scatter_rec<false>, dim3((unsigned)(g1 + n1)), dim3(kP3Threads),
                           lds, c->stream, (const double*)nullptr, c->rec_a, n, p, c->zref, start1, blk2,
                           cursor2, c->rec_b, (double*)nullptr);
        AMHIP_TRY(hipGetLastError());
      }
      {
        ScopedTimer t(c, AMHIP_K_DSM_SCAN);
        if ((rc = ensure_capacity(&c->bin_z, &c->bin_z_cap, 2 * (nbins + 4)))) return rc;
        uint2* bin_z = reinterpret_cast<uint2*>(c->bin_z);
        uint4* rec16 = reinterpret_cast<uint4*>(c->rec16);
        const size_t lds = (size_t)p.p3_cap * kRecWords * 4 + (3 * (size_t)p.p3_w + 32) * sizeof(uint32_t);
        AMHIP_TRY(hipFuncSetAttribute(reinterpret_cast<const void*>(k_dsm_p3_place_rec),
                                      hipFuncAttributeMaxDynamicSharedMemorySize, (int)lds));
        hipLaunchKernelGGL(k_dsm_p3_place_rec, dim3((unsigned)nk), dim3(kP3PlaceThreads), lds,
                           c->stream, c->rec_b, p, p.p3_cap, start2, c->bin_start, rec16, c->sidx, bin_z,
                           (unsigned)p.p3_cap, 0xFFFFFFFFu);
        const size_t tables = (4 * (size_t)p.p3_w + 64) * sizeof(uint32_t);
        int cap_rounds = (int)std::min<size_t>(kP3BigCap, (kLdsMaxBytes - tables) / (kRecWords * 4));
        unsigned rounds_above = kP3BigCap, reg_max = 0xFFFFFFFFu;
        p3_rounds_knob(&cap_rounds, &rounds_above, &reg_max);
        const size_t lds_big = std::max((size_t)kP3BigCap * kRecWords * 4 + (3 * (size_t)p.p3_w + 32) * sizeof(uint32_t),
                                        (size_t)cap_rounds * kRecWords * 4 + tables);
        AMHIP_TRY(hipFuncSetAttribute(reinterpret_cast<const void*>(k_dsm_p3_place_rec_big),
                                      hipFuncAttributeMaxDynamicSharedMemorySize, (int)lds_big));
        hipLaunchKernelGGL(k_dsm_p3_place_rec_big, dim3(256), dim3(kP3BigThreads), lds_big, c->stream,
                           c->rec_b, p, start2, c->bin_start, rec16, c->sidx, bin_z, big_list, cap_rounds, rounds_above, reg_max);
        AMHIP_TRY(hipGetLastError());
        c->bin_z_valid = true;
        c->pts = PtsView{nullptr, rec16, c->sidx, dev_xyz, c->zref, p.sub_x, p.sub_y};
      }
      return AMHIP_OK;
    }
    {
      ScopedTimer t(c, AMHIP_K_DSM_SCATTER);
      const size_t lds = (size_t)kP3Chunk * 28 + (3 * kP3MaxKeys + 32) * sizeof(uint32_t);
      AMHIP_TRY(hipFuncSetAttribute(reinterpret_cast<const void*>(k_dsm_p3_scatter<true>),
                                    hipFuncAttributeMaxDynamicSharedMemorySize, (int)lds));
      AMHIP_TRY(hipFuncSetAttribute(reinterpret_cast<const void*>(k_dsm_p3_scatter<false>),
                                    hipFuncAttributeMaxDynamicSharedMemorySize, (int)lds));
      const size_t g1 = (n + kP3Chunk - 1) / kP3Chunk;
      hipLaunchKernelGGL(k_dsm_p3_scatter<true>, dim3((unsigned)g1), dim3(kP3Threads), lds,
                         c->stream, dev_xyz, dev_values, n, p, start1, blk2, cursor1, c->sorted,
                         zpart);
      c->range_parts = (size_t)g1 * (kP3Threads / 64);
      hipLaunchKernelGGL(k_dsm_p3_scatter<false>, dim3((unsigned)(g1 + n1)), dim3(kP3Threads),
                         lds, c->stream, c->sorted, (const int32_t*)nullptr, n, p, start1, blk2,
                         cursor2, c->tmp_points, (double*)nullptr);
      AMHIP_TRY(hipGetLastError());
    }
    {
      ScopedTimer t(c, AMHIP_K_DSM_SCAN);
      uint2* bin_z = nullptr;
      const size_t zlds = bin_z ? 2 * (size_t)p.p3_w * sizeof(uint32_t) : 0;
      const size_t lds = (size_t)p.p3_cap * 24 + ((size_t)p.p3_w + 32) * sizeof(uint32_t) + zlds;
      AMHIP_TRY(hipFuncSetAttribute(reinterpret_cast<const void*>(k_dsm_p3_place),
                                    hipFuncAttributeMaxDynamicSharedMemorySize, (int)lds));
      const bool want_big = !(c->sort_stats_sig == geo_sig && c->host_sort_stats && c->host_sort_stats[0] == 0u) ||
                            no_launch_skips();
      c->sort_stats_sig = geo_sig;
      hipLaunchKernelGGL(k_dsm_p3_place, dim3((unsigned)nk), dim3(kP3PlaceThreads), lds,
                         c->stream, c->tmp_points, p, p.p3_cap, start2, c->bin_start, c->sorted,
                         want_big ? (unsigned)p.p3_cap : 0xFFFFFFFFu, 0xFFFFFFFFu, bin_z,
                         (const uint32_t*)big_list, c->host_sort_stats);
      const size_t tables = (4 * (size_t)p.p3_w + 64) * sizeof(uint32_t);
      int cap_rounds = (int)std::min<size_t>(kP3BigCap, (kLdsMaxBytes - tables) / 24);
      unsigned rounds_above = kP3BigCap, reg_max = 0xFFFFFFFFu;
      p3_rounds_knob(&cap_rounds, &rounds_above, &reg_max);
      const size_t lds_big = std::max((size_t)kP3BigCap * 24 + ((size_t)p.p3_w + 32) * sizeof(uint32_t) + zlds,
                                      (size_t)cap_rounds * 24 + tables);
      AMHIP_TRY(hipFuncSetAttribute(reinterpret_cast<const void*>(k_dsm_p3_place_big),
                                    hipFuncAttributeMaxDynamicSharedMemorySize, (int)lds_big));
      if (want_big)
        hipLaunchKernelGGL(k_dsm_p3_place_big, dim3(256), dim3(kP3BigThreads), lds_big, c->stream,
                           c->tmp_points, p, start2, c->bin_start, c->sorted, big_list, bin_z, cap_rounds, rounds_above, reg_max);
      c->bin_z_valid = bin_z != nullptr;
      AMHIP_TRY(hipGetLastError());
    }
  } else {
    {
      int rc;
      if ((rc = ensure_capacity(&c->rank, &c->rank_cap, n))) return rc;
      if ((rc = ensure_capacity(&c->scan_partials, &c->partial_cap, nblocks_scan + 4))) return rc;
    }
    {
      ScopedTimer t(c, AMHIP_K_MISC);
// ... 48 lines not shown
```

### aerial_mapper_amd/csrc/amhip_tuning.cc

```cpp
#include "amhip_tuning.h"

#include <cmath>
#include <cstdio>
#include <cstdlib>
#include <cstring>
#include <atomic>
#include <mutex>
#include <string>

namespace amhip {

namespace {

const char* const kKeys[] = {
    "sort_one_level", "p3_min_points", "p3_target", "p3_cap", "p3_rounds_cap", "p3_rounds_reread",
    "no_launch_skips",
    "dsm_canon_all", "knn_global_bins", "dsm_no_rough_switch", "dsm_no_subwindow", "eager_reset",
    "ortho_exact_fold", "ortho_no_prune", "no_coarse_cull", "ortho_no_tile_list",
    "no_distorted_cull", "no_distorted_prune", "distorted_square_cull",
    "session_always_copy", "session_threads", "session_scalar_sums", "session_no_partial",
    "session_verify_partial", "session_trace", "session_serial_sums",
    "gather_tj", "gather_nt", "gather_class_cap0", "gather_class_cap1", "gather_class_cap2", "f32_variant",
    "fx_theta"};

constexpr int kNumKeys = (int)(sizeof(kKeys) / sizeof(kKeys[0]));

int key_index(const char* k, size_t len) {
  for (int i = 0; i < kNumKeys; ++i)
    if (std::strlen(kKeys[i]) == len && std::memcmp(kKeys[i], k, len) == 0) return i;
  return -1;
}

struct Store {
  std::atomic<double> values[kNumKeys];
  std::once_flag env_once;
  Store() {
    for (auto& v : values) v.store(std::nan(""), std::memory_order_relaxed);
  }
  void read_env() {
    const char* e = std::getenv("AMHIP_TUNING");
    if (!e) return;
    std::string s(e);
    size_t pos = 0;
    while (pos <= s.size()) {
      size_t end = s.find(',', pos);
      if (end == std::string::npos) end = s.size();
      std::string item = s.substr(pos, end - pos);
      pos = end + 1;
      while (!item.empty() && item[0] == ' ') item.erase(0, 1);
      if (item.empty()) continue;
      const size_t eq = item.find('=');
      const std::string key = item.substr(0, eq);
      const double v = eq == std::string::npos ? 1.0 : std::atof(item.c_str() + eq + 1);
      const int k = key_index(key.data(), key.size());
      if (k < 0) {
        std::fprintf(stderr, "libaerial_mapper_hip: AMHIP_TUNING names an unknown key '%s' (ignored)\n", key.c_str());
        continue;
      }
      values[k].store(v, std::memory_order_relaxed);
    }
  }
  void ensure_env() { std::call_once(env_once, [this] { read_env(); }); }
};

Store& store() {
  static Store s;
  return s;
}

}

double tuning(const char* key, double dflt) {
  Store& s = store();
  s.ensure_env();
  const int k = key ? key_index(key, std::strlen(key)) : -1;
  if (k < 0) return dflt;
  const double v = s.values[k].load(std::memory_order_relaxed);
  return std::isnan(v) ? dflt : v;
}

bool tuning_set(const char* key, double value) {
  const int k = key ? key_index(key, std::strlen(key)) : -1;
  if (k < 0) return false;
  Store& s = store();
  s.ensure_env();
  s.values[k].store(value, std::memory_order_relaxed);
  return true;
}

}
```

### aerial_mapper_amd/hip_lib.py

```python
import ctypes as C
import os

PKG = os.path.dirname(os.path.abspath(__file__))
LIB_PATH = os.environ.get("AMHIP_LIB_PATH") or os.path.join(PKG, "lib", "libaerial_mapper_hip.so")

ABI_VERSION = 2

OK, ERR_ARG, ERR_EXACT_HIT, ERR_ALPHA_NONPOS, ERR_HIP, ERR_NO_DEVICE, ERR_NOMEM, ERR_HALO_OVERFLOW = range(8)
STATUS_NAMES = {OK: "AMHIP_OK", ERR_ARG: "AMHIP_ERR_ARG", ERR_EXACT_HIT: "AMHIP_ERR_EXACT_HIT",
                ERR_ALPHA_NONPOS: "AMHIP_ERR_ALPHA_NONPOS", ERR_HIP: "AMHIP_ERR_HIP",
                ERR_NO_DEVICE: "AMHIP_ERR_NO_DEVICE", ERR_NOMEM: "AMHIP_ERR_NOMEM",
                ERR_HALO_OVERFLOW: "AMHIP_ERR_HALO_OVERFLOW"}

(LAYER_ORTHO, LAYER_ELEVATION, LAYER_ELEVATION_ANGLE, LAYER_NUM_OBSERVATIONS,
 LAYER_OBSERVATION_INDEX, LAYER_COLORED_ORTHO) = range(6)
NUM_LAYERS = 6
LAYER_NAMES = ["ortho", "elevation", "elevation_angle", "num_observations",
               "observation_index", "colored_ortho"]

(K_DSM_BIN_COUNT, K_DSM_SCAN, K_DSM_SCATTER, K_DSM_GATHER, K_ORTHO, K_MISC,
 K_HALO_SELECT, K_STEREO) = range(8)
NUM_KERNELS = 8

DIST_NONE, DIST_RADTAN, DIST_EQUIDISTANT = 0, 1, 2

STEREO_MAX_BATCH = 16

EXPORTS = [
    "amhip_abi_version", "amhip_last_error", "amhip_make_grid", "amhip_cell_position",
    "amhip_ctx_create", "amhip_ctx_create_window", "amhip_ctx_destroy", "amhip_ctx_set_dsm_precision", "amhip_ctx_set_dsm_knn", "amhip_ctx_set_stream", "amhip_ctx_synchronize",
    "amhip_layers_reset", "amhip_layer_upload", "amhip_layer_download",
    "amhip_layer_device_ptr", "amhip_dsm_process_dev", "amhip_dsm_process",
    "amhip_ortho_from_pcl_process_dev", "amhip_ortho_from_pcl_process",
    "amhip_densify_dev", "amhip_rectify_stereo_pair_dev", "amhip_halo_select_dev", "amhip_dsm_tiled_begin_dev",
    "amhip_dsm_tiled_finish_dev", "amhip_compose_T_G_C", "amhip_ortho_backward_process_dev",
    "amhip_ortho_backward_process", "amhip_ctx_enable_timing", "amhip_ctx_timing_reset",
    "amhip_ctx_kernel_time", "amhip_kernel_name", "amhip_ctx_dsm_stats", "amhip_ctx_dsm_gather_stats", "amhip_ctx_order_after", "amhip_session_last_profile", "amhip_build_id", "amhip_set_tuning", "amhip_get_tuning", "amhip_default_dsm_precision",
    "amhip_mosaic_create", "amhip_mosaic_destroy", "amhip_mosaic_set_stream",
    "amhip_mosaic_synchronize", "amhip_mosaic_reset", "amhip_mosaic_batch",
    "amhip_mosaic_batch_dev", "amhip_mosaic_update", "amhip_mosaic_update_dev",
    "amhip_mosaic_download", "amhip_mosaic_device_ptr", "amhip_mosaic_homography",
    "amhip_camera_view_bounds",
    "amhip_session_create", "amhip_session_destroy", "amhip_session_num_windows",
    "amhip_session_context", "amhip_session_window", "amhip_session_set_always_copy",
    "amhip_session_set_dsm_precision", "amhip_session_transfer_stats",
    "amhip_session_dsm_process", "amhip_session_ortho_backward_process",
    "amhip_session_ortho_from_pcl_process",
    "amhip_io_parse_point_cloud_text", "amhip_io_download_point_cloud", "amhip_io_free",
    "amhip_layer_to_image_dev", "amhip_layer_to_image", "amhip_geotiff_write_u8",
    "amhip_grid_map_msg_bytes", "amhip_grid_map_msg_layout", "amhip_io_write_point_cloud_binary",
    "amhip_io_load_point_cloud_binary", "amhip_session_grid_map_msg", "amhip_session_layer_to_image",
    "amhip_sgbm_default_params", "amhip_sgbm_disparity_dev",
    "amhip_bm_default_params", "amhip_bm_disparity_dev",
    "amhip_sgbm_disparity_batch_dev", "amhip_bm_disparity_batch_dev", "amhip_stereo_set_pairs_in_flight",
    "amhip_stereo_default_settings", "amhip_stereo_create", "amhip_stereo_destroy", "amhip_stereo_reset",
    "amhip_stereo_add_frame", "amhip_stereo_add_frame_dev", "amhip_stereo_add_frames",
    "amhip_stereo_add_frames_dev", "amhip_stereo_cloud", "amhip_stereo_point_cloud2_dev",
    "amhip_jpeg_bound", "amhip_jpeg_encode_dev", "amhip_jpeg_write", "amhip_layer_write_jpeg",
    "amhip_session_layer_write_jpeg", "amhip_mosaic_encode_jpeg_dev", "amhip_mosaic_write_jpeg",
]


class GridDesc(C.Structure):
    _fields_ = [("rows", C.c_int32), ("cols", C.c_int32),
                ("resolution", C.c_double),
                ("length_x", C.c_double), ("length_y", C.c_double),
                ("pos_x", C.c_double), ("pos_y", C.c_double)]


class Camera(C.Structure):
    _fields_ = [("fu", C.c_double), ("fv", C.c_double),
                ("cu", C.c_double), ("cv", C.c_double),
                ("width", C.c_int32), ("height", C.c_int32),
                ("distortion", C.c_int32), ("_pad", C.c_int32),
                ("dist", C.c_double * 4)]


class MosaicDesc(C.Structure):
    _fields_ = [("width_mosaic_pixels", C.c_int32), ("height_mosaic_pixels", C.c_int32),
                ("ground_plane_elevation_m", C.c_double), ("origin", C.c_double * 3)]


class SgbmParams(C.Structure):
    _fields_ = [(n, C.c_int32) for n in (
        "min_disparity", "num_disparities", "pre_filter_cap", "uniqueness_ratio",
        "speckle_window_size", "speckle_range", "disp_12_max_diff", "p1", "p2", "block_size")]


class BmParams(C.Structure):
    _fields_ = [(n, C.c_int32) for n in (
        "min_disparity", "num_disparities", "pre_filter_cap", "pre_filter_size", "uniqueness_ratio",
        "texture_threshold", "speckle_window_size", "speckle_range", "disp_12_max_diff", "block_size")]


class StereoSettings(C.Structure):
    _fields_ = [("use_every_nth_image", C.c_uint64), ("images_need_undistortion", C.c_int32),
                ("use_bm", C.c_int32), ("_pad", C.c_int32 * 2), ("sgbm", SgbmParams), ("bm", BmParams)]


class AmhipError(RuntimeError):
    def __init__(self, status, message):
        super().__init__("%s: %s" % (STATUS_NAMES.get(status, status), message))
        self.status = status


_lib = None


def load():
    global _lib
    if _lib is not None:
        return _lib
    if not os.path.exists(LIB_PATH):
        raise ImportError(
            "%s is missing: run `python -m aerial_mapper_amd.build` "
            "(there is no CPU fallback for the hot path)" % LIB_PATH)
    try:
        import torch
    except Exception:
        pass
    lib = C.CDLL(LIB_PATH)
    vp, f64p, f32p = C.c_void_p, C.POINTER(C.c_double), C.POINTER(C.c_float)
    gp, cp = C.POINTER(GridDesc), C.POINTER(Camera)
    lib.amhip_abi_version.restype = C.c_int
    lib.amhip_last_error.restype = C.c_char_p
    lib.amhip_make_grid.restype = None
    lib.amhip_make_grid.argtypes = [C.c_double] * 5 + [gp]
    lib.amhip_cell_position.restype = None
    lib.amhip_cell_position.argtypes = [gp, C.c_int, C.c_int, f64p, f64p]
    lib.amhip_ctx_create.argtypes = [gp, C.c_int, C.POINTER(vp)]
    lib.amhip_ctx_create_window.argtypes = [gp, C.c_int, C.c_int, C.c_int, C.c_int, C.c_int,
                                            C.POINTER(vp)]
    lib.amhip_ctx_destroy.restype = None
    lib.amhip_ctx_destroy.argtypes = [vp]
    lib.amhip_ctx_set_stream.argtypes = [vp, vp]
    lib.amhip_ctx_set_dsm_precision.argtypes = [vp, C.c_int]
    lib.amhip_ctx_set_dsm_knn.argtypes = [vp, C.c_int]
    lib.amhip_ctx_synchronize.argtypes = [vp]
    lib.amhip_layers_reset.argtypes = [vp]
    lib.amhip_layer_upload.argtypes = [vp, C.c_int, vp]
    lib.amhip_layer_download.argtypes = [vp, C.c_int, vp]
    lib.amhip_layer_device_ptr.restype = vp
    lib.amhip_layer_device_ptr.argtypes = [vp, C.c_int]
    lib.amhip_dsm_process_dev.argtypes = [vp, vp, C.c_size_t, C.c_int, C.c_double, C.c_double]
    lib.amhip_dsm_process.argtypes = [vp, vp, C.c_size_t, C.c_int, C.c_double, C.c_double, vp]
    lib.amhip_ortho_from_pcl_process_dev.argtypes = [vp, vp, vp, C.c_size_t, C.c_int, C.c_int]
    lib.amhip_ortho_from_pcl_process.argtypes = [vp, vp, vp, C.c_size_t, C.c_int, C.c_int, vp]
    lib.amhip_densify_dev.argtypes = [vp, vp, C.c_size_t, vp, C.c_size_t, C.c_int, C.c_int, f64p,
                                      C.c_double, f64p, f64p, vp, vp, C.c_size_t, vp]
    lib.amhip_halo_select_dev.argtypes = [vp, vp, C.c_size_t, C.c_double, C.c_double,
                                          C.POINTER(C.c_int32), C.c_int, C.c_double, vp,
                                          C.c_size_t, vp]
    lib.amhip_dsm_tiled_begin_dev.argtypes = [vp, vp, C.c_size_t, C.c_size_t, C.c_int, C.c_double,
                                              C.c_double, C.POINTER(C.c_int32), C.c_int,
                                              C.c_double, vp, C.c_size_t, vp]
    lib.amhip_dsm_tiled_finish_dev.argtypes = [vp]
    lib.amhip_compose_T_G_C.restype = None
    lib.amhip_compose_T_G_C.argtypes = [f64p, f64p, C.c_size_t, f64p]
    lib.amhip_ortho_backward_process_dev.argtypes = [
        vp, cp, f64p, C.c_size_t, vp, C.c_size_t, C.c_size_t, C.c_int, C.c_int]
    lib.amhip_ortho_backward_process.argtypes = [
        vp, cp, f64p, C.c_size_t, C.POINTER(vp), C.POINTER(C.c_size_t), C.c_int, C.c_int,
        vp, vp, vp, vp, vp, vp]
    lib.amhip_session_create.argtypes = [gp, C.c_int, C.c_int, C.POINTER(C.c_int32), C.POINTER(vp)]
    lib.amhip_session_destroy.restype = None
    lib.amhip_session_destroy.argtypes = [vp]
    lib.amhip_session_num_windows.argtypes = [vp]
    lib.amhip_session_context.restype = vp
    lib.amhip_session_context.argtypes = [vp, C.c_int]
    lib.amhip_session_window.argtypes = [vp, C.c_int, C.POINTER(C.c_int32)]
    lib.amhip_session_set_always_copy.argtypes = [vp, C.c_int]
    lib.amhip_session_set_dsm_precision.argtypes = [vp, C.c_int]
    lib.amhip_ctx_order_after.argtypes = [vp, vp]
    lib.amhip_session_transfer_stats.argtypes = [vp, C.POINTER(C.c_uint64), C.POINTER(C.c_uint64)]
    lib.amhip_session_last_profile.argtypes = [vp, C.POINTER(C.c_double)]
    lib.amhip_session_dsm_process.argtypes = [vp, vp, C.c_size_t, C.c_int, C.c_double, C.c_double, vp]
    lib.amhip_session_ortho_from_pcl_process.argtypes = [vp, vp, vp, C.c_size_t, C.c_int, C.c_int, vp]
    lib.amhip_session_ortho_backward_process.argtypes = [
        vp, cp, f64p, C.c_size_t, C.POINTER(vp), C.POINTER(C.c_size_t), C.c_int, C.c_int,
        vp, vp, vp, vp, vp, vp]
    lib.amhip_rectify_stereo_pair_dev.argtypes = [vp, f64p, f64p, f64p, f64p, f64p, C.c_int, C.c_int,
                                                  vp, C.c_size_t, vp, C.c_size_t, f64p, f64p, vp, vp, vp, vp]
    lib.amhip_sgbm_default_params.restype = None
    lib.amhip_sgbm_default_params.argtypes = [C.POINTER(SgbmParams)]
    lib.amhip_sgbm_disparity_dev.argtypes = [vp, C.POINTER(SgbmParams), C.c_int, C.c_int,
                                             vp, C.c_size_t, vp, C.c_size_t, vp, C.c_size_t,
                                             vp, C.c_size_t, vp, C.c_size_t]
    lib.amhip_bm_default_params.restype = None
    lib.amhip_bm_default_params.argtypes = [C.POINTER(BmParams)]
    lib.amhip_bm_disparity_dev.argtypes = [vp, C.POINTER(BmParams), C.c_int, C.c_int,
                                           vp, C.c_size_t, vp, C.c_size_t, vp, C.c_size_t,
                                           vp, C.c_size_t, vp, C.c_size_t]
    batch_io = [vp, C.c_size_t, C.c_size_t] * 5
    lib.amhip_sgbm_disparity_batch_dev.argtypes = [vp, C.POINTER(SgbmParams), C.c_int, C.c_int, C.c_int] + batch_io
    lib.amhip_bm_disparity_batch_dev.argtypes = [vp, C.POINTER(BmParams), C.c_int, C.c_int, C.c_int] + batch_io
    lib.amhip_stereo_set_pairs_in_flight.argtypes = [vp, C.c_int]
    sp = C.POINTER(StereoSettings)
    lib.amhip_stereo_default_settings.restype = None
    lib.amhip_stereo_default_settings.argtypes = [sp]
    lib.amhip_stereo_create.argtypes = [vp, cp, f64p, sp, C.POINTER(vp)]
    lib.amhip_stereo_destroy.argtypes = [vp]
    lib.amhip_stereo_reset.argtypes = [vp]
    lib.amhip_stereo_add_frame.argtypes = [vp, f64p, vp, C.c_size_t, C.c_int]
    lib.amhip_stereo_add_frame_dev.argtypes = [vp, f64p, vp, C.c_size_t, C.c_int]
    lib.amhip_stereo_add_frames.argtypes = [vp, f64p, C.POINTER(vp), C.POINTER(C.c_size_t), C.c_int,
                                            C.c_size_t]
    lib.amhip_stereo_add_frames_dev.argtypes = [vp, f64p, vp, C.c_size_t, C.c_size_t, C.c_int,
                                                C.c_size_t]
    lib.amhip_stereo_cloud.argtypes = [vp, C.POINTER(vp), C.POINTER(vp), C.POINTER(C.c_size_t),
                                       C.POINTER(C.c_size_t)]
    lib.amhip_stereo_point_cloud2_dev.argtypes = [vp, C.POINTER(vp), C.POINTER(C.c_size_t)]
    lib.amhip_ctx_enable_timing.argtypes = [vp, C.c_int]
    lib.amhip_ctx_timing_reset.argtypes = [vp]
    lib.amhip_ctx_kernel_time.argtypes = [vp, C.c_int, f64p, C.POINTER(C.c_int64)]
    lib.amhip_kernel_name.restype = C.c_char_p
    lib.amhip_set_tuning.argtypes = [C.c_char_p, C.c_double]
    lib.amhip_get_tuning.restype = C.c_double
    lib.amhip_get_tuning.argtypes = [C.c_char_p, C.c_double]
    lib.amhip_default_dsm_precision.argtypes = []
    lib.amhip_build_id.restype = C.c_char_p
    lib.amhip_build_id.argtypes = []
    lib.amhip_kernel_name.argtypes = [C.c_int]
    lib.amhip_ctx_dsm_gather_stats.argtypes = [vp, C.POINTER(C.c_int64)]
    lib.amhip_ctx_dsm_stats.argtypes = [vp, C.POINTER(C.c_int64), C.POINTER(C.c_int64),
                                        C.POINTER(C.c_int32)]
    mp = C.POINTER(MosaicDesc)
    lib.amhip_mosaic_create.argtypes = [mp, cp, C.c_int, C.POINTER(vp)]
    lib.amhip_mosaic_destroy.argtypes = [vp]
    lib.amhip_mosaic_set_stream.argtypes = [vp, vp]
    lib.amhip_mosaic_synchronize.argtypes = [vp]
    lib.amhip_mosaic_reset.argtypes = [vp]
    lib.amhip_mosaic_batch.argtypes = [vp, f64p, C.c_size_t, C.POINTER(vp), C.POINTER(C.c_size_t),
                                       C.c_int, vp, vp]
    lib.amhip_mosaic_batch_dev.argtypes = [vp, f64p, C.c_size_t, vp, C.c_size_t, C.c_size_t,
                                           C.c_int]
    lib.amhip_mosaic_update.argtypes = [vp, f64p, vp, C.c_size_t, C.c_int, vp, vp]
    lib.amhip_mosaic_update_dev.argtypes = [vp, f64p, vp, C.c_size_t, C.c_int]
    lib.amhip_mosaic_download.argtypes = [vp, vp, vp]
    lib.amhip_mosaic_device_ptr.argtypes = [vp, C.POINTER(vp), C.POINTER(vp)]
    lib.amhip_mosaic_homography.argtypes = [mp, cp, f64p, C.c_int, f64p]
    lib.amhip_camera_view_bounds.argtypes = [cp, f64p]
    lib.amhip_io_parse_point_cloud_text.argtypes = [C.c_int, C.c_char_p, C.c_size_t, C.POINTER(vp),
                                                    C.POINTER(vp), C.POINTER(C.c_size_t),
                                                    C.POINTER(C.c_size_t)]
    lib.amhip_io_download_point_cloud.argtypes = [vp, vp, C.c_size_t, vp, vp]
    lib.amhip_io_free.argtypes = [vp]
    u8p = C.POINTER(C.c_uint8)
    lib.amhip_layer_to_image_dev.argtypes = [vp, C.c_int, C.c_int, C.c_float, C.c_float, vp, C.c_size_t]
    lib.amhip_layer_to_image.argtypes = [vp, C.c_int, C.c_int, C.c_float, C.c_float, vp, C.c_size_t]
    lib.amhip_geotiff_write_u8.argtypes = [C.c_char_p, vp, C.c_int, C.c_int, C.c_size_t, C.c_int,
                                           f64p, C.c_int, C.c_int]
    lib.amhip_grid_map_msg_bytes.restype = C.c_size_t
    lib.amhip_grid_map_msg_bytes.argtypes = [gp, C.c_char_p, C.c_int, C.POINTER(C.c_char_p)]
    lib.amhip_grid_map_msg_layout.argtypes = [gp, C.c_uint64, C.c_char_p, C.c_int,
                                              C.POINTER(C.c_char_p), vp, C.c_size_t,
                                              C.POINTER(C.c_size_t)]
    lib.amhip_io_write_point_cloud_binary.argtypes = [C.c_char_p, vp, vp, C.c_size_t]
    lib.amhip_io_load_point_cloud_binary.argtypes = [C.c_int, C.c_char_p, C.POINTER(vp),
                                                     C.POINTER(vp), C.POINTER(C.c_size_t)]
    lib.amhip_session_grid_map_msg.argtypes = [vp, C.c_uint64, C.c_char_p, C.c_int,
                                               C.POINTER(C.c_char_p), C.POINTER(C.c_int32),
                                               C.POINTER(vp), vp, C.c_size_t,
                                               C.POINTER(C.c_size_t)]
    lib.amhip_session_layer_to_image.argtypes = [vp, C.c_int, C.c_int, C.c_float, C.c_float, vp,
                                                 C.c_size_t]
    lib.amhip_jpeg_bound.restype = C.c_size_t
    lib.amhip_jpeg_bound.argtypes = [C.c_int, C.c_int, C.c_int]
    lib.amhip_jpeg_encode_dev.argtypes = [vp, vp, C.c_size_t, C.c_int, C.c_int, C.c_int, C.c_int, vp,
                                          C.c_size_t, C.POINTER(C.c_size_t)]
    lib.amhip_jpeg_write.argtypes = [vp, C.c_char_p, vp, C.c_int, C.c_size_t, C.c_int, C.c_int, C.c_int,
                                     C.c_int]
    lib.amhip_layer_write_jpeg.argtypes = [vp, C.c_int, C.c_int, C.c_float, C.c_float, C.c_int, C.c_char_p]
    lib.amhip_session_layer_write_jpeg.argtypes = [vp, C.c_int, C.c_int, C.c_float, C.c_float, C.c_int,
                                                   C.c_char_p]
    lib.amhip_mosaic_encode_jpeg_dev.argtypes = [vp, C.c_int, vp, C.c_size_t, C.POINTER(C.c_size_t)]
    lib.amhip_mosaic_write_jpeg.argtypes = [vp, C.c_int, C.c_char_p]
    del u8p
    missing = [name for name in EXPORTS if not hasattr(lib, name)]
    if missing:
        raise ImportError("libaerial_mapper_hip.so lacks %s (stale build?)" % missing)
    if lib.amhip_abi_version() != ABI_VERSION:
        raise ImportError("libaerial_mapper_hip.so ABI %d != expected %d"
                          % (lib.amhip_abi_version(), ABI_VERSION))
    _lib = lib
    return lib


def set_tuning(key, value=1.0):
    check(load().amhip_set_tuning(key.encode(), float("nan") if value is None else float(value)))


def tuning_env(**knobs):
    return {"AMHIP_TUNING": ",".join("%s=%s" % (k, v) for k, v in knobs.items())}


def build_id():
    return load().amhip_build_id().decode()


def last_error():
    return load().amhip_last_error().decode("utf-8", "replace")


def check(status):
    if status != OK:
        raise AmhipError(status, last_error())
    return status


def make_grid(length_x, length_y, resolution, pos_x=0.0, pos_y=0.0):
    g = GridDesc()
    load().amhip_make_grid(length_x, length_y, resolution, pos_x, pos_y, C.byref(g))
    return g


def cell_position(g, i, j):
    x, y = C.c_double(), C.c_double()
    load().amhip_cell_position(C.byref(g), i, j, C.byref(x), C.byref(y))
    return x.value, y.value
```

### aerial_mapper_amd/mapper.py

```python
import ctypes as C

import numpy as np

from . import hip_lib as L


class GridMapSettings(object):

    def __init__(self, center_easting=0.0, center_northing=0.0, delta_easting=0.0,
                 delta_northing=0.0, resolution=1.0):
        self.center_easting = center_easting
        self.center_northing = center_northing
        self.delta_easting = delta_easting
        self.delta_northing = delta_northing
        self.resolution = resolution


class AerialGridMap(object):

    def __init__(self, settings, device=0, window=None):
        self.settings = settings
        lib = L.load()
        self.grid = L.make_grid(settings.delta_easting, settings.delta_northing,
                                settings.resolution, settings.center_easting,
                                settings.center_northing)
        if window is None:
            window = (0, 0, self.grid.rows, self.grid.cols)
        self.window = tuple(int(v) for v in window)
        h = C.c_void_p()
        L.check(lib.amhip_ctx_create_window(C.byref(self.grid), self.window[0], self.window[1],
                                            self.window[2], self.window[3], int(device),
                                            C.byref(h)))
        self._h = h
        self._lib = lib
        self.device = int(device)

    def close(self):
        if getattr(self, "_h", None):
            self._lib.amhip_ctx_destroy(self._h)
            self._h = None

    def __del__(self):
        try:
            self.close()
        except Exception:
            pass

    def __enter__(self):
        return self

    def __exit__(self, *a):
        self.close()

    @property
    def rows(self):
        return self.window[2]

    @property
    def cols(self):
        return self.window[3]

    @property
    def num_cells(self):
        return self.window[2] * self.window[3]

    @property
    def handle(self):
        return self._h

    @staticmethod
    def _layer_id(layer):
        return L.LAYER_NAMES.index(layer) if isinstance(layer, str) else int(layer)

    def get(self, layer, out=None):
        if out is None:
            out = np.empty((self.cols, self.rows), np.float32)
        assert out.dtype == np.float32 and out.shape == (self.cols, self.rows) and out.flags.c_contiguous
        L.check(self._lib.amhip_layer_download(self._h, self._layer_id(layer),
                                               out.ctypes.data))
        return out

    def host_mirror(self, layer):
        if not hasattr(self, "_mirrors"):
            self._mirrors, self._mirror_fresh = {}, set()
        buf = self._mirrors.get(layer)
        if buf is None:
            buf = self._mirrors[layer] = np.zeros((self.cols, self.rows), np.float32)
            buf.fill(0.0)
        if layer not in self._mirror_fresh:
            self.get(layer, out=buf)
            self._mirror_fresh.add(layer)
        return buf

    def _touched(self, *layers):
        if hasattr(self, "_mirror_fresh"):
            if layers:
                self._mirror_fresh.difference_update(layers)
            else:
                self._mirror_fresh.clear()

    def set(self, layer, values):
        self._touched(layer)
        a = np.ascontiguousarray(values, np.float32)
        assert a.shape == (self.cols, self.rows), a.shape
        L.check(self._lib.amhip_layer_upload(self._h, self._layer_id(layer), a.ctypes.data))

    def device_ptr(self, layer):
        self._touched(layer)
        self._external = getattr(self, "_external", set()) | {layer}
        return self._lib.amhip_layer_device_ptr(self._h, self._layer_id(layer))

    def as_torch(self, layer):
        import torch
        ptr = self.device_ptr(layer)
        n = self.num_cells

        class _Holder(object):
            pass

        holder = _Holder()
        holder.__cuda_array_interface__ = {
            "shape": (self.cols, self.rows), "typestr": "<f4",
            "data": (int(ptr), False), "version": 2}
        holder._keepalive = self
        assert n > 0
        return torch.as_tensor(holder, device="cuda:%d" % self.device)

    def reset(self):
        self._touched()
        L.check(self._lib.amhip_layers_reset(self._h))

    def set_stream(self, stream_handle):
        L.check(self._lib.amhip_ctx_set_stream(self._h, C.c_void_p(stream_handle or 0)))
        self._stream_handle = int(stream_handle or 0)

    def wait_for_torch(self, tensor):
        import torch
        cur = torch.cuda.current_stream(tensor.device)
        if int(cur.cuda_stream) == 0 or int(cur.cuda_stream) != getattr(self, "_stream_handle", 0):
            cur.synchronize()

    def torch_waits(self):
        import torch
        cur = torch.cuda.current_stream(torch.device("cuda", self.device))
        if int(cur.cuda_stream) == 0 or int(cur.cuda_stream) != getattr(self, "_stream_handle", 0):
            L.check(self._lib.amhip_ctx_order_after(self._h, C.c_void_p(int(cur.cuda_stream))))

    def synchronize(self):
        L.check(self._lib.amhip_ctx_synchronize(self._h))

    def set_dsm_precision(self, exact):
        L.check(self._lib.amhip_ctx_set_dsm_precision(self._h, 1 if exact else 0))

    def set_dsm_knn(self, k):
        L.check(self._lib.amhip_ctx_set_dsm_knn(self._h, int(k)))

    def enable_timing(self, on=True):
        L.check(self._lib.amhip_ctx_enable_timing(self._h, int(bool(on))))

    def timing_reset(self):
        L.check(self._lib.amhip_ctx_timing_reset(self._h))

    def kernel_times(self):
        out = {}
        for k in range(L.NUM_KERNELS):
            ms, n = C.c_double(), C.c_int64()
            L.check(self._lib.amhip_ctx_kernel_time(self._h, k, C.byref(ms), C.byref(n)))
            out[self._lib.amhip_kernel_name(k).decode()] = (ms.value, n.value)
        return out

    def dsm_stats(self):
        a, b, c = C.c_int64(), C.c_int64(), C.c_int32()
        L.check(self._lib.amhip_ctx_dsm_stats(self._h, C.byref(a), C.byref(b), C.byref(c)))
        return {"points_binned": a.value, "num_bins": b.value, "bin_cells": c.value}

    def dsm_gather_stats(self):
        out = (C.c_int64 * 8)()
        L.check(self._lib.amhip_ctx_dsm_gather_stats(self._h, out))
        v = [int(x) for x in out]
        return {"tiles": v[7], "sparse_list": v[0], "class1": v[1], "class2": v[2],
                "beyond_lds": v[3], "f32_to_fp64": v[4] + v[5], "f32_to_fp64_beyond": v[6]}


def _is_torch(x):
    return type(x).__module__.startswith("torch")


class DsmSettings(object):

    def __init__(self, interpolation_radius=1, adaptive_interpolation=False,
                 center_easting=0.0, center_northing=0.0, use_multi_threads=True):
        self.interpolation_radius = int(interpolation_radius)
        self.adaptive_interpolation = adaptive_interpolation
        self.center_easting = center_easting
        self.center_northing = center_northing
        self.use_multi_threads = use_multi_threads


class Dsm(object):

    def __init__(self, settings, map):
        if map is None:
            raise L.AmhipError(L.ERR_ARG, "CHECK(map) (dsm.cc:22)")
        self.settings = settings

    def process(self, point_cloud, map, sync=True):
        if map is None:
            raise L.AmhipError(L.ERR_ARG, "CHECK(map) (dsm.cc:194)")
        s = self.settings
        lib = L.load()
        if _is_torch(point_cloud):
            assert point_cloud.is_cuda and point_cloud.dtype.is_floating_point
            assert point_cloud.element_size() == 8 and point_cloud.is_contiguous()
            n = point_cloud.numel() // 3
            map.wait_for_torch(point_cloud)
            map._touched("elevation")
            L.check(lib.amhip_dsm_process_dev(
                map.handle, C.c_void_p(point_cloud.data_ptr()), n,
                s.interpolation_radius, s.center_easting, s.center_northing))
            if sync:
                map.synchronize()
            else:
                map.torch_waits()
            return
        pts = np.ascontiguousarray(point_cloud, np.float64).reshape(-1, 3)
        if pts.shape[0] == 0:
            return
        if "elevation" in getattr(map, "_external", ()):
            map._touched("elevation")
        elev = map.host_mirror("elevation")
        L.check(lib.amhip_dsm_process(map.handle, pts.ctypes.data, pts.shape[0],
                                      s.interpolation_radius, s.center_easting,
                                      s.center_northing, elev.ctypes.data))


class OrthoSettings(object):

    def __init__(self, show_orthomosaic_opencv=True, save_orthomosaic_jpg=True,
                 orthomosaic_jpg_filename="", orthomosaic_elevation_m=0.0,
                 use_digital_elevation_map=True, colored_ortho=False,
                 use_multi_threads=True):
        self.show_orthomosaic_opencv = show_orthomosaic_opencv
        self.save_orthomosaic_jpg = save_orthomosaic_jpg
        self.orthomosaic_jpg_filename = orthomosaic_jpg_filename
        self.orthomosaic_elevation_m = orthomosaic_elevation_m
        self.use_digital_elevation_map = use_digital_elevation_map
        self.colored_ortho = colored_ortho
        self.use_multi_threads = use_multi_threads


class NCamera(object):

    def __init__(self, fu, fv, cu, cv, width, height, distortion=L.DIST_NONE,
                 dist=(0.0, 0.0, 0.0, 0.0), T_C_B=(0, 0, 0, 1, 0, 0, 0)):
        self.camera = L.Camera()
        self.camera.fu, self.camera.fv, self.camera.cu, self.camera.cv = fu, fv, cu, cv
        self.camera.width, self.camera.height = int(width), int(height)
        self.camera.distortion = int(distortion)
        for k in range(4):
            self.camera.dist[k] = float(dist[k])
        self.T_C_B = np.asarray(T_C_B, np.float64).reshape(7).copy()


def compose_T_G_C(T_G_Bs, T_C_B):
    T = np.ascontiguousarray(T_G_Bs, np.float64).reshape(-1, 7)
    tcb = np.ascontiguousarray(T_C_B, np.float64).reshape(7)
    out = np.empty_like(T)
    f64p = C.POINTER(C.c_double)
    L.load().amhip_compose_T_G_C(T.ctypes.data_as(f64p), tcb.ctypes.data_as(f64p),
                                 T.shape[0], out.ctypes.data_as(f64p))
    return out


class OrthoBackwardGrid(object):

    def __init__(self, ncameras, settings, map=None):
        if ncameras is None:
            raise L.AmhipError(L.ERR_ARG, "CHECK(ncameras_) (ortho-backward-grid.cc:27)")
        if settings.use_multi_threads and map is None:
            raise L.AmhipError(L.ERR_ARG, "map must not be null")
        self.ncameras = ncameras
        self.settings = settings

    def process(self, T_G_Bs, images, map, sync=True):
        T_G_Bs = np.ascontiguousarray(T_G_Bs, np.float64).reshape(-1, 7)
        F = T_G_Bs.shape[0]
        if F == 0:
            raise L.AmhipError(L.ERR_ARG, "CHECK(!T_G_Bs.empty())")
        if len(images) != F:
            raise L.AmhipError(L.ERR_ARG, "CHECK(T_G_Bs.size() == images.size())")
        if map is None:
            raise L.AmhipError(L.ERR_ARG, "CHECK(map)")
        lib = L.load()
        map._touched("elevation_angle", "observation_index", "num_observations", "ortho",
                     "colored_ortho")
        cam = self.ncameras.camera
        colored = bool(self.settings.colored_ortho)
        T_G_C = compose_T_G_C(T_G_Bs, self.ncameras.T_C_B)
        f64p = C.POINTER(C.c_double)
        if _is_torch(images):
            assert images.is_cuda and images.is_contiguous() and images.element_size() == 1
            ch = 3 if images.dim() == 4 else 1
            row = cam.width * ch
            frame = row * cam.height
            assert images.shape[1] == cam.height and images.shape[2] == cam.width
            map.wait_for_torch(images)
            L.check(lib.amhip_ortho_backward_process_dev(
                map.handle, C.byref(cam), T_G_C.ctypes.data_as(f64p), F,
                C.c_void_p(images.data_ptr()), frame, row, ch, int(colored)))
            if sync:
                map.synchronize()
            return
        ch = 3 if colored else 1
        ptrs = (C.c_void_p * F)()
        steps = (C.c_size_t * F)()
        keep = []
        for k, im in enumerate(images):
            im = np.asarray(im)
            if im.dtype != np.uint8 or im.strides[-1] != 1 or \
                    (im.ndim == 3 and (im.shape[2] != 3 or im.strides[1] != 3)):
                im = np.ascontiguousarray(im, np.uint8)
            if (im.ndim == 3) != colored:
                raise L.AmhipError(L.ERR_ARG, "colored_ortho needs 8UC3 frames, gray needs 8UC1")
            keep.append(im)
            ptrs[k] = im.ctypes.data
            steps[k] = im.strides[0]
        L.check(lib.amhip_ortho_backward_process(
# ... 636 lines not shown
```

### include/aerial_mapper_hip.h

```cpp
#ifndef AERIAL_MAPPER_HIP_H_
#define AERIAL_MAPPER_HIP_H_

#include <stddef.h>
#include <stdint.h>

#ifdef __cplusplus
extern "C" {
#endif

#define AMHIP_ABI_VERSION 2

typedef enum amhip_status {
  AMHIP_OK = 0,
  AMHIP_ERR_ARG = 1,
  AMHIP_ERR_EXACT_HIT = 2,
  AMHIP_ERR_ALPHA_NONPOS = 3,
  AMHIP_ERR_HIP = 4,
  AMHIP_ERR_NO_DEVICE = 5,
  AMHIP_ERR_NOMEM = 6,
  AMHIP_ERR_HALO_OVERFLOW = 7
} amhip_status;

typedef struct amhip_grid_desc {
  int32_t rows;
// ... 165 lines not shown
int amhip_layer_to_image_dev(amhip_ctx* ctx, int layer, int bgr, float lower, float upper,
                             uint8_t* dev_image, size_t step);
int amhip_layer_to_image(amhip_ctx* ctx, int layer, int bgr, float lower, float upper,
                         uint8_t* host_image, size_t step);

size_t amhip_jpeg_bound(int width, int height, int channels);
int amhip_jpeg_encode_dev(amhip_ctx* ctx, const uint8_t* dev_pixels, size_t step, int width, int height,
                          int channels, int quality, uint8_t* dev_out, size_t cap, size_t* bytes);
int amhip_jpeg_write(amhip_ctx* ctx, const char* filename, const uint8_t* pixels, int on_device,
                     size_t step, int width, int height, int channels, int quality);
int amhip_layer_write_jpeg(amhip_ctx* ctx, int layer, int bgr, float lower, float upper, int quality,
                           const char* filename);

int amhip_geotiff_write_u8(const char* filename, const uint8_t* pixels, int width, int height,
                           size_t step, int bands, const double* geotransform, int utm_zone,
                           int northern);

size_t amhip_grid_map_msg_bytes(const amhip_grid_desc* grid, const char* frame_id, int num_layers,
                                const char* const* layer_names);
int amhip_grid_map_msg_layout(const amhip_grid_desc* grid, uint64_t stamp_ns, const char* frame_id,
                              int num_layers, const char* const* layer_names, uint8_t* out,
                              size_t cap, size_t* payload_offsets);

int amhip_io_write_point_cloud_binary(const char* filename, const double* host_xyz,
                                      const int32_t* host_intensities, size_t n);
int amhip_io_load_point_cloud_binary(int device, const char* filename, double** dev_xyz,
                                     int32_t** dev_intensities, size_t* num_points);


typedef enum amhip_kernel {
  AMHIP_K_DSM_BIN_COUNT = 0,
  AMHIP_K_DSM_SCAN = 1,
  AMHIP_K_DSM_SCATTER = 2,
  AMHIP_K_DSM_GATHER = 3,
  AMHIP_K_ORTHO = 4,
  AMHIP_K_MISC = 5,
  AMHIP_K_HALO_SELECT = 6,
  AMHIP_K_STEREO = 7,
  AMHIP_NUM_KERNELS = 8
} amhip_kernel;

int amhip_rectify_stereo_pair_dev(amhip_ctx* ctx, const double* K, const double* R_G_C1,
                                  const double* R_G_C2, const double* t_G_C1, const double* t_G_C2,
                                  int width, int height, const uint8_t* dev_left, size_t left_step,
                                  const uint8_t* dev_right, size_t right_step, double* R_G_C_out,
                                  double* baseline_out, float* dev_maps, uint8_t* dev_rect_left,
                                  uint8_t* dev_rect_right, uint8_t* dev_mask);

typedef struct amhip_sgbm_params {
  int32_t min_disparity, num_disparities, pre_filter_cap, uniqueness_ratio,
          speckle_window_size, speckle_range, disp_12_max_diff, p1, p2, block_size;
} amhip_sgbm_params;
void amhip_sgbm_default_params(amhip_sgbm_params* out);
int amhip_sgbm_disparity_dev(amhip_ctx* ctx, const amhip_sgbm_params* p, int width, int height,
                             const uint8_t* dev_left, size_t left_step,
                             const uint8_t* dev_right, size_t right_step,
                             const uint8_t* dev_mask, size_t mask_step,
                             float* dev_disparity, size_t disp_step,
                             int16_t* dev_raw, size_t raw_step);

typedef struct amhip_bm_params {
  int32_t min_disparity, num_disparities, pre_filter_cap, pre_filter_size, uniqueness_ratio,
          texture_threshold, speckle_window_size, speckle_range, disp_12_max_diff, block_size;
} amhip_bm_params;
void amhip_bm_default_params(amhip_bm_params* out);
int amhip_bm_disparity_dev(amhip_ctx* ctx, const amhip_bm_params* p, int width, int height,
                           const uint8_t* dev_left, size_t left_step,
                           const uint8_t* dev_right, size_t right_step,
                           const uint8_t* dev_mask, size_t mask_step,
                           float* dev_disparity, size_t disp_step,
                           int16_t* dev_raw, size_t raw_step);

#define AMHIP_STEREO_MAX_BATCH 16
int amhip_sgbm_disparity_batch_dev(amhip_ctx* ctx, const amhip_sgbm_params* p, int width, int height,
                                   int batch,
                                   const uint8_t* dev_left, size_t left_step, size_t left_batch_stride,
                                   const uint8_t* dev_right, size_t right_step, size_t right_batch_stride,
                                   const uint8_t* dev_mask, size_t mask_step, size_t mask_batch_stride,
                                   float* dev_disparity, size_t disp_step, size_t disp_batch_stride,
                                   int16_t* dev_raw, size_t raw_step, size_t raw_batch_stride);
int amhip_bm_disparity_batch_dev(amhip_ctx* ctx, const amhip_bm_params* p, int width, int height,
                                 int batch,
                                 const uint8_t* dev_left, size_t left_step, size_t left_batch_stride,
                                 const uint8_t* dev_right, size_t right_step, size_t right_batch_stride,
                                 const uint8_t* dev_mask, size_t mask_step, size_t mask_batch_stride,
                                 float* dev_disparity, size_t disp_step, size_t disp_batch_stride,
                                 int16_t* dev_raw, size_t raw_step, size_t raw_batch_stride);

typedef struct amhip_stereo amhip_stereo;
typedef struct amhip_stereo_settings {
  uint64_t use_every_nth_image;
  int32_t images_need_undistortion;
  int32_t use_bm;
  int32_t _pad[2];
  amhip_sgbm_params sgbm;
  amhip_bm_params bm;
} amhip_stereo_settings;
void amhip_stereo_default_settings(amhip_stereo_settings* out);

int amhip_stereo_create(amhip_ctx* ctx, const amhip_camera* cam, const double* T_C_B7,
                        const amhip_stereo_settings* settings, amhip_stereo** out);
int amhip_stereo_destroy(amhip_stereo* stereo);
int amhip_stereo_reset(amhip_stereo* stereo);
int amhip_stereo_set_pairs_in_flight(amhip_stereo* stereo, int n);

int amhip_stereo_add_frame(amhip_stereo* stereo, const double* T_G_B7, const uint8_t* host_image,
                           size_t step, int channels);
int amhip_stereo_add_frame_dev(amhip_stereo* stereo, const double* T_G_B7, const uint8_t* dev_image,
                               size_t step, int channels);

int amhip_stereo_add_frames(amhip_stereo* stereo, const double* T_G_B7xF,
                            const uint8_t* const* host_images, const size_t* steps, int channels,
                            size_t F);
int amhip_stereo_add_frames_dev(amhip_stereo* stereo, const double* T_G_B7xF,
                                const uint8_t* dev_frames, size_t frame_stride, size_t row_step,
                                int channels, size_t F);

int amhip_stereo_cloud(amhip_stereo* stereo, const double** dev_xyz, const int32_t** dev_intensities,
                       size_t* n, size_t* pairs);

int amhip_stereo_point_cloud2_dev(amhip_stereo* stereo, const void** dev_data, size_t* bytes);

typedef struct amhip_session amhip_session;
int amhip_session_create(const amhip_grid_desc* grid, int tiles_i, int tiles_j,
                         const int32_t* devices, amhip_session** out);
void amhip_session_destroy(amhip_session* s);
int amhip_session_num_windows(const amhip_session* s);
amhip_ctx* amhip_session_context(amhip_session* s, int window);
int amhip_session_window(const amhip_session* s, int window, int32_t* i0_j0_rows_cols);
int amhip_session_set_always_copy(amhip_session* s, int on);
int amhip_session_set_dsm_precision(amhip_session* s, int mode);
int amhip_session_transfer_stats(const amhip_session* s, uint64_t* uploaded_bytes,
                                 uint64_t* downloaded_bytes);
int amhip_session_last_profile(const amhip_session* s, double* out8);
int amhip_session_dsm_process(amhip_session* s, const double* host_xyz, size_t n, int radius_sq,
                              double center_easting, double center_northing, float* elevation);
int amhip_session_ortho_from_pcl_process(amhip_session* s, const double* host_xyz,
                                         const int32_t* host_intensities, size_t n, int radius_sq,
                                         int adaptive, float* ortho);
int amhip_session_ortho_backward_process(
    amhip_session* s, const amhip_camera* cam, const double* host_T_G_C, size_t F,
    const uint8_t* const* images, const size_t* steps, int channels, int colored,
    const float* elevation, float* elevation_angle, float* observation_index,
    float* num_observations, float* ortho, float* colored_ortho);

int amhip_ctx_enable_timing(amhip_ctx* ctx, int on);
int amhip_ctx_timing_reset(amhip_ctx* ctx);
int amhip_ctx_kernel_time(amhip_ctx* ctx, int kernel, double* total_ms,
                          int64_t* launches);
const char* amhip_kernel_name(int kernel);

int amhip_ctx_dsm_stats(amhip_ctx* ctx, int64_t* points_binned,
                        int64_t* num_bins, int32_t* bin_cells);

int amhip_ctx_dsm_gather_stats(amhip_ctx* ctx, int64_t* out8);

int amhip_ctx_order_after(amhip_ctx* ctx, void* other_stream);

int amhip_session_grid_map_msg(amhip_session* s, uint64_t stamp_ns, const char* frame_id,
                               int num_layers, const char* const* layer_names,
                               const int32_t* layer_ids, const float* const* host_layers,
                               uint8_t* out, size_t cap, size_t* written);
int amhip_session_layer_to_image(amhip_session* s, int layer, int bgr, float lower, float upper,
                                 uint8_t* host_image, size_t step);
int amhip_session_layer_write_jpeg(amhip_session* s, int layer, int bgr, float lower, float upper,
                                   int quality, const char* filename);

int amhip_set_tuning(const char* key, double value);
double amhip_get_tuning(const char* key, double dflt);
int amhip_default_dsm_precision(void);

const char* amhip_build_id(void);

#ifdef __cplusplus
}
#endif
#endif
```

Baseline: 18070.

## Add run-table based three-pass DSM sort that avoids global atomic scatter

Adds a new three-pass DSM point-sort pipeline. Each chunk writes its sorted keys contiguously and records per-key run offsets and counts in tables. Later passes find source rows by binary search over prefix-summed run tables (cached in LDS when small) instead of scattering through global atomic cursors. The aim is to replace scattered global writes and atomics with coalesced chunk writes. The cost is indirect gathers, extra scan kernels and table memory. The path is enabled by default for non-windowed, non-record, non-split inputs, and a query API reports which sort pipeline ran.

New measurement: 19030, median of 6. 5.4% higher.

```diff
diff --git a/aerial_mapper_amd/csrc/amhip_api.hip b/aerial_mapper_amd/csrc/amhip_api.hip
--- a/aerial_mapper_amd/csrc/amhip_api.hip
+++ b/aerial_mapper_amd/csrc/amhip_api.hip
@@ -752,6 +752,7 @@
   c->win_j0 = j0;
   c->win_rows = rows;
   c->win_cols = cols;
+  c->windowed = rows != grid->rows || cols != grid->cols;
   c->cells = static_cast<size_t>(rows) * static_cast<size_t>(cols);
   {
     c->dsm_exact = amhip_default_dsm_precision() == AMHIP_DSM_EXACT ? 1 : 0;
@@ -1584,4 +1585,10 @@
   return AMHIP_OK;
 }
 
-}
+int amhip_ctx_dsm_sort_pipeline(amhip_ctx* h, int32_t* pipeline) {
+  if (!h || !pipeline) return arg_fail("amhip_ctx_dsm_sort_pipeline: null argument");
+  *pipeline = h->impl.last_sort_pipeline;
+  return AMHIP_OK;
+}
+
+}
diff --git a/aerial_mapper_amd/csrc/amhip_common.h b/aerial_mapper_amd/csrc/amhip_common.h
--- a/aerial_mapper_amd/csrc/amhip_common.h
+++ b/aerial_mapper_amd/csrc/amhip_common.h
@@ -146,6 +146,7 @@
   amhip_grid_desc grid;
   int win_i0 = 0, win_j0 = 0;
   int win_rows = 0, win_cols = 0;
+  bool windowed = false;
   int device = 0;
   hipStream_t own_stream = nullptr;
   hipStream_t stream = nullptr;
@@ -233,6 +234,7 @@
   int64_t last_points_binned = 0;
   int64_t last_num_bins = 0;
   int32_t last_bin_cells = 0;
+  int last_sort_pipeline = -1;
   int64_t last_ntiles = 0;
   uint32_t* aux_zero_words = nullptr;
   int aux_nzero = 0;
diff --git a/aerial_mapper_amd/csrc/amhip_sort.hip b/aerial_mapper_amd/csrc/amhip_sort.hip
--- a/aerial_mapper_amd/csrc/amhip_sort.hip
+++ b/aerial_mapper_amd/csrc/amhip_sort.hip
@@ -412,13 +412,23 @@
 }
 
 
-template <bool kFirst>
+struct RunTabs {
+  uint32_t* run1;
+  uint32_t* pre1;
+  uint32_t* seg1;
+  uint32_t* run2;
+  uint32_t* pre2;
+  uint32_t g1, r1s, p1s;
+};
+constexpr int kRunsCache = 2048;
+
+template <bool kFirst, bool kRuns = false>
 __device__ __forceinline__ void p3_scatter_body(const unsigned vb, const double* __restrict__ src,
                                                 const int32_t* __restrict__ values, size_t n,
                                                 const DsmParams& p, const uint32_t* __restrict__ start1,
                                                 const uint32_t* __restrict__ blk2,
                                                 uint32_t* __restrict__ cursor, double* __restrict__ dst,
-                                                double* __restrict__ zpart) {
+                                                double* __restrict__ zpart, const RunTabs rt = RunTabs{}) {
   extern __shared__ double s_pts[];
   uint32_t* s_dest = reinterpret_cast<uint32_t*>(s_pts + 3 * kP3Chunk);
   uint32_t* s_cnt = s_dest + kP3Chunk;
@@ -428,6 +438,7 @@
   const int tid = threadIdx.x;
   int nkeys;
   size_t c0, c1;
+  uint32_t part = 0, seg = 0, nseg = 0;
   if (kFirst) {
     c0 = (size_t)vb * kP3Chunk;
     c1 = min(c0 + (size_t)kP3Chunk, n);
@@ -444,8 +455,55 @@
     c0 = (size_t)start1[lo] + (size_t)(b - blk2[lo]) * kP3Chunk;
     c1 = min(c0 + (size_t)kP3Chunk, (size_t)start1[lo + 1]);
     nkeys = p.p3_n2;
-    cursor += (size_t)lo * p.p3_n2;
-  }
+    if (!kRuns) cursor += (size_t)lo * p.p3_n2;
+    if (kRuns) {
+      part = lo;
+      seg = b - blk2[lo];
+      nseg = blk2[lo + 1] - blk2[lo];
+    }
+  }
+  uint32_t* const s_rpre = reinterpret_cast<uint32_t*>(s_pts);
+  uint32_t* const s_rsrc = s_rpre + kRunsCache;
+  const uint32_t* prow = nullptr;
+  const uint32_t* rrow = nullptr;
+  uint32_t l0 = 0, ca = 0, nr = 0;
+  bool cached = false;
+  if (kRuns && !kFirst) {
+    if (c1 <= c0) return;
+    prow = rt.pre1 + (size_t)part * rt.p1s;
+    rrow = rt.run1 + (size_t)part * rt.r1s;
+    const uint32_t* srow = rt.seg1 + (size_t)part * rt.p1s;
+    l0 = seg * (uint32_t)kP3Chunk;
+    ca = min(srow[seg], rt.g1 - 1u);
+    const uint32_t cb = seg + 1u < nseg ? min(srow[seg + 1u], rt.g1 - 1u) : rt.g1 - 1u;
+    nr = cb >= ca ? cb - ca + 1u : 1u;
+    cached = nr <= (uint32_t)kRunsCache;
+    if (cached) {
+      for (uint32_t i = tid; i < nr; i += kP3Threads) {
+        const uint32_t c = ca + i, pre = prow[c];
+        const uint32_t at = max(pre, l0);
+        s_rpre[i] = at - l0;
+        s_rsrc[i] = c * (uint32_t)kP3Chunk + (rrow[c] >> 16) + (at - pre);
+      }
+    }
+  }
+  auto run_src = [&](uint32_t j) -> size_t {
+    uint32_t a = 0, b = nr;
+    if (cached) {
+      while (b - a > 1u) {
+        const uint32_t mid = (a + b) >> 1;
+        if (s_rpre[mid] <= j) a = mid; else b = mid;
+      }
+      return (size_t)s_rsrc[a] + (j - s_rpre[a]);
+    }
+    const uint32_t g = l0 + j;
+    while (b - a > 1u) {
+      const uint32_t mid = (a + b) >> 1;
+      if (prow[ca + mid] <= g) a = mid; else b = mid;
+    }
+    const uint32_t c = ca + a, pre = prow[c];
+    return (size_t)c * kP3Chunk + (rrow[c] >> 16) + (g - min(pre, g));
+  };
   if (tid < kP3MaxKeys) s_cnt[tid] = 0;
   __syncthreads();
   double px[kP3PerThread], py[kP3PerThread], pz[kP3PerThread];
@@ -454,7 +512,8 @@
   if (c1 <= c0) return;
 #pragma unroll
   for (int k = 0; k < kP3PerThread; ++k) {
-    const size_t ld = min(c0 + tid + (size_t)k * kP3Threads, c1 - 1);
+    size_t ld = min(c0 + tid + (size_t)k * kP3Threads, c1 - 1);
+    if (kRuns && !kFirst) ld = min(run_src((uint32_t)(ld - c0)), n - 1);
     px[k] = src[3 * ld + 0];
     py[k] = src[3 * ld + 1];
     pz[k] = src[3 * ld + 2];
@@ -498,7 +557,14 @@
     const unsigned ex = block_excl_scan<kP3Threads>(c, &total, s_scan);
     if (tid < nkeys) {
       s_off[tid] = ex;
-      if (c) my_base = atomicAdd(&cursor[tid], c);
+      if (kRuns) {
+        if (kFirst)
+          rt.run1[(size_t)tid * rt.r1s + vb] = (ex << 16) | c;
+        else
+          rt.run2[(size_t)blk2[part] * nkeys + (size_t)tid * nseg + seg] = (ex << 16) | c;
+      } else if (c) {
+        my_base = atomicAdd(&cursor[tid], c);
+      }
     }
     if (tid == 0) s_scan[23] = total;
   }
@@ -511,12 +577,17 @@
       s_pts[3 * q + 0] = px[k];
       s_pts[3 * q + 1] = py[k];
       s_pts[3 * q + 2] = pz[k];
-      s_dest[q] = slot[k];
-    }
-  }
-  if (tid < nkeys) s_base[tid] = my_base;
+      if (!kRuns) s_dest[q] = slot[k];
+    }
+  }
+  if (!kRuns && tid < nkeys) s_base[tid] = my_base;
   __syncthreads();
   const uint32_t ne = 3u * s_scan[23];
+  if (kRuns) {
+    double* out = dst + 3 * (kFirst ? c0 : (size_t)start1[part] + (size_t)seg * kP3Chunk);
+    for (uint32_t e = tid; e < ne; e += kP3Threads) out[e] = s_pts[e];
+    return;
+  }
   for (uint32_t e = tid; e < ne; e += kP3Threads) {
     const uint32_t q = e / 3u;
     const uint32_t d = s_dest[q];
@@ -534,22 +605,193 @@
   p3_scatter_body<kFirst>(blockIdx.x, src, values, n, p, start1, blk2, cursor, dst, zpart);
 }
 
+__global__ void __launch_bounds__(kP3Threads)
+k_dsm_runs_sort1(const double* __restrict__ src, const int32_t* __restrict__ values, size_t n,
+                 DsmParams p, double* __restrict__ dst, double* __restrict__ zpart, RunTabs rt) {
+  p3_scatter_body<true, true>(blockIdx.x, src, values, n, p, nullptr, nullptr, nullptr, dst, zpart, rt);
+}
+
+__global__ void __launch_bounds__(kP3Threads)
+k_dsm_runs_sort2(const double* __restrict__ src, size_t n, DsmParams p,
+                 const uint32_t* __restrict__ start1, const uint32_t* __restrict__ blk2,
+                 double* __restrict__ dst, RunTabs rt) {
+  p3_scatter_body<false, true>(blockIdx.x, src, nullptr, n, p, start1, blk2, nullptr, dst, nullptr, rt);
+}
+
+__global__ void __launch_bounds__(1024)
+k_dsm_runs_scan1(RunTabs rt, int n1, uint32_t* __restrict__ tot1, uint32_t* __restrict__ start1,
+                 uint32_t* __restrict__ blk2, unsigned chunk, SortAux aux, unsigned* __restrict__ ticket) {
+  __shared__ unsigned lds[1024 / 64 + 1];
+  __shared__ unsigned s_last;
+  const int tid = threadIdx.x;
+  const uint32_t k1 = blockIdx.x;
+  const uint32_t* row = rt.run1 + (size_t)k1 * rt.r1s;
+  uint32_t* out = rt.pre1 + (size_t)k1 * rt.p1s;
+  uint32_t* seg = rt.seg1 + (size_t)k1 * rt.p1s;
+  unsigned carry = 0;
+  for (uint32_t base = 0; base < rt.g1; base += 4096u) {
+    const uint32_t i0 = base + 4u * tid;
+    uint4 w = make_uint4(0u, 0u, 0u, 0u);
+    if (i0 < rt.g1) w = *reinterpret_cast<const uint4*>(row + i0);
+    unsigned v[4] = {w.x & 0xFFFFu, w.y & 0xFFFFu, w.z & 0xFFFFu, w.w & 0xFFFFu};
+#pragma unroll
+    for (int q = 0; q < 4; ++q)
+      if (i0 + q >= rt.g1) v[q] = 0u;
+    unsigned total;
+    unsigned run = carry + block_excl_scan<1024>(v[0] + v[1] + v[2] + v[3], &total, lds);
+    unsigned pre[4];
+#pragma unroll
+    for (int q = 0; q < 4; ++q) {
+      pre[q] = run;
+      if (v[q]) {
+        const unsigned m = (run + chunk - 1u) / chunk;
+        if (m * chunk < run + v[q] && m < rt.g1) seg[m] = i0 + q;
+      }
+      run += v[q];
+    }
+    if (i0 < rt.g1) *reinterpret_cast<uint4*>(out + i0) = make_uint4(pre[0], pre[1], pre[2], pre[3]);
+    carry += total;
+  }
+  __syncthreads();
+  if (tid == 0) {
+    out[rt.g1] = carry;
+    tot1[k1] = carry;
+    __threadfence();
+    s_last = atomicAdd(ticket, 1u) == gridDim.x - 1u ? 1u : 0u;
+  }
+  __syncthreads();
+  if (!s_last) return;
+  __threadfence();
+  if (tid == 0) *ticket = 0u;
+  aux_reset(aux);
+  const unsigned t = tid < n1 ? tot1[tid] : 0u;
+  unsigned total;
+  const unsigned ex = block_excl_scan<1024>(t, &total, lds);
+  if (tid < n1) start1[tid] = ex;
+  if (tid == 0) start1[n1] = total;
+  const unsigned exb = block_excl_scan<1024>((t + chunk - 1u) / chunk, &total, lds);
+  if (tid < n1) blk2[tid] = exb;
+  if (tid == 0) blk2[n1] = total;
+}
+
+__global__ void __launch_bounds__(1024)
+k_dsm_runs_scan2(RunTabs rt, uint32_t* __restrict__ cnt, int n1, int n2, const uint32_t* __restrict__ blk2) {
+  const int nk = n1 * n2;
+  const int lane = threadIdx.x & 63, wid = threadIdx.x >> 6;
+  for (int sp = (int)blockIdx.x * 16 + wid; sp < nk; sp += (int)gridDim.x * 16) {
+    const int k1 = sp / n2, k2 = sp - k1 * n2;
+    const uint32_t b0 = blk2[k1], nseg = blk2[k1 + 1] - b0;
+    const size_t at = (size_t)b0 * n2 + (size_t)k2 * nseg;
+    const uint32_t* row = rt.run2 + at;
+    uint32_t* out = rt.pre2 + at;
+    unsigned run = 0;
+    for (uint32_t i0 = 0; i0 < nseg; i0 += 256u) {
+      unsigned v[4];
+#pragma unroll
+      for (int q = 0; q < 4; ++q) {
+        const uint32_t i = i0 + 64u * q + lane;
+        v[q] = i < nseg ? row[i] & 0xFFFFu : 0u;
+      }
+#pragma unroll
+      for (int q = 0; q < 4; ++q) {
+        const uint32_t i = i0 + 64u * q + lane;
+        const unsigned incl = wave_incl_scan(v[q], lane);
+        if (i < nseg) out[i] = run + incl - v[q];
+        run += __shfl(incl, 63, 64);
+      }
+    }
+    if (lane == 0) cnt[sp] = run;
+  }
+}
+
+__global__ void __launch_bounds__(1024)
+k_dsm_runs_plan2(const uint32_t* __restrict__ cnt, int n1, int n2,
+                 uint32_t* __restrict__ start2, uint32_t* __restrict__ cursor2,
+                 uint32_t* __restrict__ start1, uint32_t* __restrict__ cursor1,
+                 uint32_t* __restrict__ blk2, unsigned cap_small, unsigned cap_big,
+                 uint32_t* __restrict__ big_list, unsigned chunk) {
+  p3_scan_body(cnt, n1, n2, start2, cursor2, start1, cursor1, blk2, cap_small, cap_big, big_list, chunk, nullptr);
+}
+
 __device__ __forceinline__ uint32_t place_zkey(double z) {
   const uint32_t b = __float_as_uint((float)z);
   return (b >> 31) ? ~b : (b | 0x80000000u);
 }
-template <int THREADS, int PER>
+constexpr int kPlaceRunsCache = 512;
+template <bool kRuns>
+struct PlaceSource {
+  const uint32_t* pre;
+  const uint32_t* run;
+  const uint32_t* s_pre;
+  const uint32_t* s_run;
+  uint32_t nseg, base, g0;
+  bool cached;
+  __device__ __forceinline__ void init(const RunTabs& rt, const uint32_t* __restrict__ start1,
+                                       const uint32_t* __restrict__ blk2, int n2, int k1, int k2,
+                                       uint32_t g0_, uint32_t* s_cache, int threads) {
+    if (!kRuns) return;
+    const uint32_t b0 = blk2[k1];
+    nseg = blk2[k1 + 1] - b0;
+    const size_t at = (size_t)b0 * n2 + (size_t)k2 * nseg;
+    pre = rt.pre2 + at;
+    run = rt.run2 + at;
+    base = start1[k1];
+    g0 = g0_;
+    cached = nseg <= (uint32_t)kPlaceRunsCache;
+    s_pre = s_cache;
+    s_run = s_cache + kPlaceRunsCache;
+    if (cached)
+      for (uint32_t i = threadIdx.x; i < nseg; i += threads) {
+        s_cache[i] = pre[i];
+        s_cache[kPlaceRunsCache + i] = run[i];
+      }
+  }
+  __device__ __forceinline__ void expand(uint32_t* s_rows, uint32_t cnt, int threads) const {
+    for (uint32_t r = threadIdx.x; r < nseg; r += threads) {
+      const uint32_t b = s_pre[r], w = s_run[r];
+      const uint32_t row = base + r * (uint32_t)kP3Chunk + (w >> 16);
+      for (uint32_t q = 0, len = w & 0xFFFFu; q < len && b + q < cnt; ++q) s_rows[b + q] = row + q;
+    }
+  }
+  __device__ __forceinline__ size_t operator()(size_t idx) const {
+    if (!kRuns) return idx;
+    const uint32_t j = (uint32_t)idx - g0;
+    uint32_t a = 0, b = nseg;
+    if (cached) {
+      while (b - a > 1u) {
+        const uint32_t mid = (a + b) >> 1;
+        if (s_pre[mid] <= j) a = mid; else b = mid;
+      }
+      return (size_t)base + (size_t)a * kP3Chunk + (s_run[a] >> 16) + (j - min(s_pre[a], j));
+    }
+    while (b - a > 1u) {
+      const uint32_t mid = (a + b) >> 1;
+      if (pre[mid] <= j) a = mid; else b = mid;
+    }
+    return (size_t)base + (size_t)a * kP3Chunk + (run[a] >> 16) + (j - min(pre[a], j));
+  }
+};
+struct PlaceRuns {
+  RunTabs rt;
+  const uint32_t* start1;
+  const uint32_t* blk2;
+  size_t n;
+};
+
+template <int THREADS, int PER, bool kRuns = false>
 __device__ __forceinline__ void place_subpartition(const double* __restrict__ src, const DsmParams& p,
                                                    int cap, const uint32_t* __restrict__ start2,
                                                    uint32_t* __restrict__ bin_start,
                                                    double* __restrict__ sorted, int sp,
                                                    unsigned skip_lo, unsigned skip_hi,
-                                                   uint2* __restrict__ bin_z) {
+                                                   uint2* __restrict__ bin_z,
+                                                   const PlaceRuns pr = PlaceRuns{}) {
   extern __shared__ double s_pts[];
   uint32_t* s_bins = reinterpret_cast<uint32_t*>(s_pts + 3 * cap);
   uint32_t* s_scan = s_bins + p.p3_w;
   uint32_t* s_zlo = s_scan + 24;
   uint32_t* s_zhi = s_zlo + p.p3_w;
+  uint32_t* s_cache = s_scan + 24 + (bin_z ? 2 * p.p3_w : 0);
   const int tid = threadIdx.x;
   const int k1 = sp / p.p3_n2, k2 = sp - k1 * p.p3_n2;
   const int rr = k2 / p.p3_c;
@@ -567,16 +809,26 @@
       s_zhi[k] = 0u;
     }
   }
+  PlaceSource<kRuns> at;
+  at.init(pr.rt, pr.start1, pr.blk2, p.p3_n2, k1, k2, g0, s_cache, THREADS);
+  auto row_of = [&](size_t idx) -> size_t { return kRuns ? min(at(idx), pr.n - 1) : idx; };
   __syncthreads();
   if ((g1 - g0) > skip_lo && (g1 - g0) <= skip_hi) return;
   const bool in_lds = (int)(g1 - g0) <= cap && cap <= THREADS * PER;
+  const bool mapped = kRuns && in_lds && at.cached;
+  const uint32_t* const s_rows = reinterpret_cast<const uint32_t*>(s_pts);
+  if (mapped) {
+    at.expand(reinterpret_cast<uint32_t*>(s_pts), g1 - g0, THREADS);
+    __syncthreads();
+  }
   double px[PER], py[PER], pz[PER];
   int pb[PER];
   if (in_lds) {
     if (g1 > g0) {
 #pragma unroll
       for (int k = 0; k < PER; ++k) {
-        const size_t ld = min(g0 + tid + (uint32_t)k * THREADS, g1 - 1);
+        const uint32_t at_k = min(g0 + tid + (uint32_t)k * THREADS, g1 - 1);
+        const size_t ld = mapped ? min((size_t)s_rows[at_k - g0], pr.n - 1) : row_of(at_k);
         px[k] = src[3 * ld + 0];
         py[k] = src[3 * ld + 1];
         pz[k] = src[3 * ld + 2];
@@ -601,7 +853,8 @@
   } else {
     for (uint32_t idx = g0 + tid; idx < g1; idx += THREADS) {
       int bx, by;
-      point_bin_xy(p, src[3 * (size_t)idx + 0], src[3 * (size_t)idx + 1], &bx, &by);
+      const size_t ld = row_of(idx);
+      point_bin_xy(p, src[3 * ld + 0], src[3 * ld + 1], &bx, &by);
       atomicAdd(&s_bins[bx - bx0], 1u);
     }
   }
@@ -630,9 +883,10 @@
   __syncthreads();
   if (!in_lds) {
     for (uint32_t idx = g0 + tid; idx < g1; idx += THREADS) {
-      const double x = src[3 * (size_t)idx + 0];
-      const double y = src[3 * (size_t)idx + 1];
-      const double z = src[3 * (size_t)idx + 2];
+      const size_t ld = row_of(idx);
+      const double x = src[3 * ld + 0];
+      const double y = src[3 * ld + 1];
+      const double z = src[3 * ld + 2];
       int bx, by;
       point_bin_xy(p, x, y, &bx, &by);
       const size_t o = (size_t)g0 + atomicAdd(&s_bins[bx - bx0], 1u);
@@ -668,12 +922,13 @@
 }
 
 
-template <int THREADS, bool kRec, int PER>
+template <int THREADS, bool kRec, int PER, bool kRuns = false>
 __device__ __forceinline__ void place_rounds(const void* __restrict__ src_v, const DsmParams& p, int cap,
                                              const uint32_t* __restrict__ start2,
                                              uint32_t* __restrict__ bin_start, double* __restrict__ sorted,
                                              uint4* __restrict__ rec16, uint32_t* __restrict__ sidx,
-                                             uint2* __restrict__ bin_z, int sp) {
+                                             uint2* __restrict__ bin_z, int sp,
+                                             const PlaceRuns pr = PlaceRuns{}) {
   extern __shared__ double s_pts_raw[];
   constexpr int kWordsPer = kRec ? 5 : 6;
   constexpr int kRegs = PER > 0 ? PER : 1;
@@ -683,6 +938,7 @@
   uint32_t* s_scan = s_cur + p.p3_w;
   uint32_t* s_zlo = s_scan + 24;
   uint32_t* s_zhi = s_zlo + p.p3_w;
+  uint32_t* s_cache = s_zhi + p.p3_w;
   const double* srcd = reinterpret_cast<const double*>(src_v);
   const uint32_t* srcw = reinterpret_cast<const uint32_t*>(src_v);
   const int tid = threadIdx.x;
@@ -700,11 +956,14 @@
       s_zlo[k] = 0xFFFFFFFFu;
       s_zhi[k] = 0u;
     }
-  __syncthreads();
-  auto bin_of = [&](uint32_t idx) -> int {
-    if (kRec) return div_by((int)(srcw[(size_t)kRecWords * idx] & 0xFFFFu), p.B, p.mul_B) - bx0;
+  PlaceSource<kRuns> at;
+  at.init(pr.rt, pr.start1, pr.blk2, p.p3_n2, k1, k2, g0, s_cache, THREADS);
+  auto row_of = [&](size_t idx) -> size_t { return kRuns ? min(at(idx), pr.n - 1) : idx; };
+  __syncthreads();
+  auto bin_of = [&](size_t ld) -> int {
+    if (kRec) return div_by((int)(srcw[(size_t)kRecWords * ld] & 0xFFFFu), p.B, p.mul_B) - bx0;
     int bx, by;
-    point_bin_xy(p, srcd[3 * (size_t)idx + 0], srcd[3 * (size_t)idx + 1], &bx, &by);
+    point_bin_xy(p, srcd[3 * ld + 0], srcd[3 * ld + 1], &bx, &by);
     return bx - bx0;
   };
   double rx[kRegs], ry[kRegs], rz[kRegs];
@@ -714,7 +973,7 @@
     if (g1 > g0) {
 #pragma unroll
       for (int k = 0; k < kRegs; ++k) {
-        const size_t ld = min(g0 + tid + (uint32_t)k * THREADS, g1 - 1);
+        const size_t ld = row_of(min(g0 + tid + (uint32_t)k * THREADS, g1 - 1));
         if (kRec) {
 #pragma unroll
           for (int t = 0; t < kRecWords; ++t) rw[k][t] = srcw[(size_t)kRecWords * ld + t];
@@ -746,7 +1005,8 @@
       }
     }
   } else {
-    for (uint32_t idx = g0 + tid; idx < g1; idx += THREADS) {
+    for (uint32_t i = g0 + tid; i < g1; i += THREADS) {
+      const size_t idx = row_of(i);
       const int b = bin_of(idx);
       atomicAdd(&s_bins[b], 1u);
       if (bin_z) {
@@ -819,7 +1079,8 @@
         }
       }
     } else {
-      for (uint32_t idx = g0 + tid; idx < g1; idx += THREADS) {
+      for (uint32_t i = g0 + tid; i < g1; i += THREADS) {
+        const size_t idx = row_of(i);
         const int bb = bin_of(idx);
         if (bb < lo_bin || bb >= hi_bin) continue;
         const uint32_t q = atomicAdd(&s_cur[bb], 1u);
@@ -883,6 +1144,40 @@
     else
       place_subpartition<kP3BigThreads, kP3BigPer>(src, p, kP3BigCap, start2, bin_start, sorted, sp, 0u,
                                                    0u, bin_z);
+    __syncthreads();
+  }
+}
+
+__global__ void __launch_bounds__(kP3PlaceThreads)
+k_dsm_runs_place(const double* __restrict__ src, DsmParams p, int cap,
+                 const uint32_t* __restrict__ start2, uint32_t* __restrict__ bin_start,
+                 double* __restrict__ sorted, unsigned skip_lo, unsigned skip_hi,
+                 uint2* __restrict__ bin_z, const uint32_t* __restrict__ big_list,
+                 unsigned* __restrict__ host_big, PlaceRuns pr) {
+  if (host_big && blockIdx.x == 0 && threadIdx.x == 0) host_big[0] = big_list[0];
+  place_subpartition<kP3PlaceThreads, kP3PlacePer, true>(src, p, cap, start2, bin_start, sorted,
+                                                         (int)blockIdx.x, skip_lo, skip_hi, bin_z, pr);
+}
+
+__global__ void __launch_bounds__(kP3BigThreads)
+k_dsm_runs_place_big(const double* __restrict__ src, DsmParams p,
+                     const uint32_t* __restrict__ start2, uint32_t* __restrict__ bin_start,
+                     double* __restrict__ sorted, const uint32_t* __restrict__ big_list,
+                     uint2* __restrict__ bin_z, int cap_rounds, unsigned rounds_above, unsigned reg_max,
+                     PlaceRuns pr) {
+  const unsigned count = big_list[0];
+  for (unsigned k = blockIdx.x; k < count; k += gridDim.x) {
+    const int sp = (int)big_list[1 + k];
+    const uint32_t cnt = start2[sp + 1] - start2[sp];
+    if (cnt > rounds_above && cnt <= min(reg_max, (unsigned)(kP3BigThreads * kP3RoundsPer)))
+      place_rounds<kP3BigThreads, false, kP3RoundsPer, true>(src, p, cap_rounds, start2, bin_start, sorted,
+                                                             nullptr, nullptr, bin_z, sp, pr);
+    else if (cnt > rounds_above)
+      place_rounds<kP3BigThreads, false, 0, true>(src, p, cap_rounds, start2, bin_start, sorted, nullptr,
+                                                  nullptr, bin_z, sp, pr);
+    else
+      place_subpartition<kP3BigThreads, kP3BigPer, true>(src, p, kP3BigCap, start2, bin_start, sorted, sp,
+                                                         0u, 0u, bin_z, pr);
     __syncthreads();
   }
 }
@@ -1443,6 +1738,104 @@
 static int dsm_sort_impl(Ctx* c, const double* dev_xyz, const int32_t* dev_values, size_t n,
                          const DsmParams& p, unsigned long long* zrange, const SortSplit* split);
 
+static int dsm_sort_runs(Ctx* c, const double* dev_xyz, const int32_t* dev_values, size_t n,
+                         const DsmParams& p, double* zpart, const SortAux& aux, unsigned long long geo_sig) {
+  const int n1 = p.p3_n1, n2 = p.p3_n2, nk = n1 * n2;
+  const size_t g1 = (n + kP3Chunk - 1) / kP3Chunk;
+  const size_t r1s = (g1 + 3) & ~(size_t)3, p1s = r1s + 4;
+  auto up4 = [](size_t w) { return (w + 3) & ~(size_t)3; };
+  const size_t plan_words = up4(4 * (size_t)nk + 4 * (size_t)n1 + 64);
+  const size_t rows2 = (g1 + (size_t)n1) * (size_t)n2;
+  const size_t ws_words = plan_words + up4((size_t)n1) + (size_t)n1 * (r1s + 2 * p1s) + 2 * up4(rows2) + 16;
+  int rc;
+  if ((rc = ensure_capacity(&c->tmp_points, &c->tmp_points_cap, 3 * n))) return rc;
+  if ((rc = ensure_capacity(&c->stripe_ws, &c->stripe_ws_cap, ws_words))) return rc;
+  uint32_t* cnt = c->stripe_ws;
+  uint32_t* start2 = cnt + nk;
+  uint32_t* cursor2 = start2 + nk + 1;
+  uint32_t* start1 = cursor2 + nk;
+  uint32_t* cursor1 = start1 + n1 + 1;
+  uint32_t* blk2 = cursor1 + n1;
+  uint32_t* big_list = blk2 + n1 + 1;
+  uint32_t* tot1 = c->stripe_ws + plan_words;
+  RunTabs rt;
+  rt.run1 = tot1 + up4((size_t)n1);
+  rt.pre1 = rt.run1 + (size_t)n1 * r1s;
+  rt.seg1 = rt.pre1 + (size_t)n1 * p1s;
+  rt.run2 = rt.seg1 + (size_t)n1 * p1s;
+  rt.pre2 = rt.run2 + up4(rows2);
+  rt.g1 = (uint32_t)g1;
+  rt.r1s = (uint32_t)r1s;
+  rt.p1s = (uint32_t)p1s;
+  const size_t lds_sort = (size_t)kP3Chunk * 28 + (3 * kP3MaxKeys + 32) * sizeof(uint32_t);
+  static_assert(2 * kRunsCache * sizeof(uint32_t) <= (size_t)kP3Chunk * 24, "the run table lies in the points' image");
+  AMHIP_TRY(hipFuncSetAttribute(reinterpret_cast<const void*>(k_dsm_runs_sort1),
+                                hipFuncAttributeMaxDynamicSharedMemorySize, (int)lds_sort));
+  AMHIP_TRY(hipFuncSetAttribute(reinterpret_cast<const void*>(k_dsm_runs_sort2),
+                                hipFuncAttributeMaxDynamicSharedMemorySize, (int)lds_sort));
+  {
+    ScopedTimer t(c, AMHIP_K_DSM_SCATTER);
+    hipLaunchKernelGGL(k_dsm_runs_sort1, dim3((unsigned)g1), dim3(kP3Threads), lds_sort, c->stream,
+                       dev_xyz, dev_values, n, p, c->sorted, zpart, rt);
+    c->range_parts = g1 * (kP3Threads / 64);
+    AMHIP_TRY(hipGetLastError());
+  }
+  {
+    ScopedTimer t(c, AMHIP_K_DSM_BIN_COUNT);
+    hipLaunchKernelGGL(k_dsm_runs_scan1, dim3((unsigned)n1), dim3(1024), 0, c->stream, rt, n1, tot1,
+                       start1, blk2, (unsigned)kP3Chunk, aux, c->dev_tickets + 2);
+    c->aux_done = true;
+    AMHIP_TRY(hipGetLastError());
+  }
+  {
+    ScopedTimer t(c, AMHIP_K_DSM_SCATTER);
+    hipLaunchKernelGGL(k_dsm_runs_sort2, dim3((unsigned)(g1 + n1)), dim3(kP3Threads), lds_sort, c->stream,
+                       c->sorted, n, p, start1, blk2, c->tmp_points, rt);
+    AMHIP_TRY(hipGetLastError());
+  }
+  {
+    ScopedTimer t(c, AMHIP_K_DSM_BIN_COUNT);
+    const unsigned grid = (unsigned)std::min<size_t>(((size_t)nk + 15) / 16, 2048);
+    hipLaunchKernelGGL(k_dsm_runs_scan2, dim3(grid), dim3(1024), 0, c->stream, rt, cnt, n1, n2,
+                       (const uint32_t*)blk2);
+    hipLaunchKernelGGL(k_dsm_runs_plan2, dim3(1), dim3(1024), 0, c->stream, (const uint32_t*)cnt, n1, n2,
+                       start2, cursor2, start1, cursor1, blk2, (unsigned)p.p3_cap, (unsigned)kP3BigCap,
+                       big_list, (unsigned)kP3Chunk);
+    AMHIP_TRY(hipGetLastError());
+  }
+  {
+    ScopedTimer t(c, AMHIP_K_DSM_SCAN);
+    const PlaceRuns pr = {rt, start1, blk2, n};
+    uint2* bin_z = nullptr;
+    const size_t cache = 2 * (size_t)kPlaceRunsCache * sizeof(uint32_t);
+    const size_t lds = (size_t)p.p3_cap * 24 + ((size_t)p.p3_w + 32) * sizeof(uint32_t) + cache;
+    AMHIP_TRY(hipFuncSetAttribute(reinterpret_cast<const void*>(k_dsm_runs_place),
+                                  hipFuncAttributeMaxDynamicSharedMemorySize, (int)lds));
+    const bool want_big = !(c->sort_stats_sig == geo_sig && c->host_sort_stats && c->host_sort_stats[0] == 0u) ||
+                          no_launch_skips();
+    c->sort_stats_sig = geo_sig;
+    hipLaunchKernelGGL(k_dsm_runs_place, dim3((unsigned)nk), dim3(kP3PlaceThreads), lds, c->stream,
+                       c->tmp_points, p, p.p3_cap, start2, c->bin_start, c->sorted,
+                       want_big ? (unsigned)p.p3_cap : 0xFFFFFFFFu, 0xFFFFFFFFu, bin_z,
+                       (const uint32_t*)big_list, c->host_sort_stats, pr);
+    const size_t tables = (4 * (size_t)p.p3_w + 64) * sizeof(uint32_t) + cache;
+    int cap_rounds = (int)std::min<size_t>(kP3BigCap, (kLdsMaxBytes - tables) / 24);
+    unsigned rounds_above = kP3BigCap, reg_max = 0xFFFFFFFFu;
+    p3_rounds_knob(&cap_rounds, &rounds_above, &reg_max);
+    const size_t lds_big = std::max((size_t)kP3BigCap * 24 + ((size_t)p.p3_w + 32) * sizeof(uint32_t) + cache,
+                                    (size_t)cap_rounds * 24 + tables);
+    AMHIP_TRY(hipFuncSetAttribute(reinterpret_cast<const void*>(k_dsm_runs_place_big),
+                                  hipFuncAttributeMaxDynamicSharedMemorySize, (int)lds_big));
+    if (want_big)
+      hipLaunchKernelGGL(k_dsm_runs_place_big, dim3(256), dim3(kP3BigThreads), lds_big, c->stream,
+                         c->tmp_points, p, start2, c->bin_start, c->sorted, big_list, bin_z, cap_rounds,
+                         rounds_above, reg_max, pr);
+    c->bin_z_valid = false;
+    AMHIP_TRY(hipGetLastError());
+  }
+  return AMHIP_OK;
+}
+
 int dsm_sort(Ctx* c, const double* dev_xyz, const int32_t* dev_values, size_t n,
              const DsmParams& p, unsigned long long* zrange, const SortSplit* split) {
   const int rc = dsm_sort_impl(c, dev_xyz, dev_values, n, p, zrange, split);
@@ -1487,6 +1880,7 @@
 
   const bool force_one_level = force_one_level_;
   const bool three_pass = p.p3_n1 > 0 && !force_one_level;
+  c->last_sort_pipeline = AMHIP_SORT_ONE_LEVEL;
   if (split && split->phase == 1 && !three_pass)
     return halo_select_run(c, dev_xyz, split->n_prefix, split->hp, split->halo_out,
                            split->halo_counts);
@@ -1500,6 +1894,10 @@
     const size_t g_a = count_grid(n_a), g_b = n > n_a ? count_grid(n - n_a) : 0;
     const size_t gcount = g_a + g_b;
     int rc;
+    const bool runs = !rec && !split && !c->windowed && n <= ((size_t)1 << 27) && n1 <= kP3MaxKeys &&
+                      n2 <= kP3MaxKeys && p.p3_w <= 2048 && tuning("sort_runs", 1.0) != 0.0;
+    c->last_sort_pipeline = runs ? AMHIP_SORT_RUNS : AMHIP_SORT_COUNT;
+    if (runs) return dsm_sort_runs(c, dev_xyz, dev_values, n, p, zpart, aux, geo_sig);
     if (rec) {
       if ((rc = ensure_capacity(&c->rec_a, &c->rec_a_cap, (size_t)kRecWords * n + 16))) return rc;
       if ((rc = ensure_capacity(&c->rec_b, &c->rec_b_cap, (size_t)kRecWords * n + 16))) return rc;
diff --git a/aerial_mapper_amd/csrc/amhip_tuning.cc b/aerial_mapper_amd/csrc/amhip_tuning.cc
--- a/aerial_mapper_amd/csrc/amhip_tuning.cc
+++ b/aerial_mapper_amd/csrc/amhip_tuning.cc
@@ -14,7 +14,7 @@
 
 const char* const kKeys[] = {
     "sort_one_level", "p3_min_points", "p3_target", "p3_cap", "p3_rounds_cap", "p3_rounds_reread",
-    "no_launch_skips",
+    "no_launch_skips", "sort_runs",
     "dsm_canon_all", "knn_global_bins", "dsm_no_rough_switch", "dsm_no_subwindow", "eager_reset",
     "ortho_exact_fold", "ortho_no_prune", "no_coarse_cull", "ortho_no_tile_list",
     "no_distorted_cull", "no_distorted_prune", "distorted_square_cull",
diff --git a/aerial_mapper_amd/hip_lib.py b/aerial_mapper_amd/hip_lib.py
--- a/aerial_mapper_amd/hip_lib.py
+++ b/aerial_mapper_amd/hip_lib.py
@@ -35,7 +35,7 @@
     "amhip_densify_dev", "amhip_rectify_stereo_pair_dev", "amhip_halo_select_dev", "amhip_dsm_tiled_begin_dev",
     "amhip_dsm_tiled_finish_dev", "amhip_compose_T_G_C", "amhip_ortho_backward_process_dev",
     "amhip_ortho_backward_process", "amhip_ctx_enable_timing", "amhip_ctx_timing_reset",
-    "amhip_ctx_kernel_time", "amhip_kernel_name", "amhip_ctx_dsm_stats", "amhip_ctx_dsm_gather_stats", "amhip_ctx_order_after", "amhip_session_last_profile", "amhip_build_id", "amhip_set_tuning", "amhip_get_tuning", "amhip_default_dsm_precision",
+    "amhip_ctx_kernel_time", "amhip_kernel_name", "amhip_ctx_dsm_stats", "amhip_ctx_dsm_sort_pipeline", "amhip_ctx_dsm_gather_stats", "amhip_ctx_order_after", "amhip_session_last_profile", "amhip_build_id", "amhip_set_tuning", "amhip_get_tuning", "amhip_default_dsm_precision",
     "amhip_mosaic_create", "amhip_mosaic_destroy", "amhip_mosaic_set_stream",
     "amhip_mosaic_synchronize", "amhip_mosaic_reset", "amhip_mosaic_batch",
     "amhip_mosaic_batch_dev", "amhip_mosaic_update", "amhip_mosaic_update_dev",
@@ -224,6 +224,7 @@
     lib.amhip_ctx_dsm_gather_stats.argtypes = [vp, C.POINTER(C.c_int64)]
     lib.amhip_ctx_dsm_stats.argtypes = [vp, C.POINTER(C.c_int64), C.POINTER(C.c_int64),
                                         C.POINTER(C.c_int32)]
+    lib.amhip_ctx_dsm_sort_pipeline.argtypes = [vp, C.POINTER(C.c_int32)]
     mp = C.POINTER(MosaicDesc)
     lib.amhip_mosaic_create.argtypes = [mp, cp, C.c_int, C.POINTER(vp)]
     lib.amhip_mosaic_destroy.argtypes = [vp]
diff --git a/aerial_mapper_amd/mapper.py b/aerial_mapper_amd/mapper.py
--- a/aerial_mapper_amd/mapper.py
+++ b/aerial_mapper_amd/mapper.py
@@ -172,7 +172,11 @@
     def dsm_stats(self):
         a, b, c = C.c_int64(), C.c_int64(), C.c_int32()
         L.check(self._lib.amhip_ctx_dsm_stats(self._h, C.byref(a), C.byref(b), C.byref(c)))
-        return {"points_binned": a.value, "num_bins": b.value, "bin_cells": c.value}
+        s = C.c_int32()
+        L.check(self._lib.amhip_ctx_dsm_sort_pipeline(self._h, C.byref(s)))
+        pipeline = {0: "one-level", 1: "count", 2: "runs"}.get(s.value)
+        return {"points_binned": a.value, "num_bins": b.value, "bin_cells": c.value,
+                "sort_pipeline": pipeline}
 
     def dsm_gather_stats(self):
         out = (C.c_int64 * 8)()
diff --git a/include/aerial_mapper_hip.h b/include/aerial_mapper_hip.h
--- a/include/aerial_mapper_hip.h
+++ b/include/aerial_mapper_hip.h
@@ -341,6 +341,10 @@
 
 int amhip_ctx_dsm_stats(amhip_ctx* ctx, int64_t* points_binned,
                         int64_t* num_bins, int32_t* bin_cells);
+#define AMHIP_SORT_ONE_LEVEL 0
+#define AMHIP_SORT_COUNT 1
+#define AMHIP_SORT_RUNS 2
+int amhip_ctx_dsm_sort_pipeline(amhip_ctx* ctx, int32_t* pipeline);
 
 int amhip_ctx_dsm_gather_stats(amhip_ctx* ctx, int64_t* out8);
 
```
